# HannesStark/3DInfomax

Hardware: AMD Instinct MI355X
Metric: molecules/sec pretraining step (PNA+Net3D, QM9-50k); PNA-agg HBM GB/s vs peak (higher is better)
Workload: dtype f32

## Files before the change

3dinfomax_amd/csrc/bn.hip:

```cpp
#include <stdlib.h>

#include <atomic>

#include "common.h"
#include "peer.h"

namespace i3d {

constexpr int MAX_PARTIAL_BLOCKS = 256;
static int partial_blocks() { return MAX_PARTIAL_BLOCKS; }
constexpr int RU = 4;

struct Chunking {
    int tpr;
    int rl;
    int rpb;
    int nblk;
    int ncolblk;
    int cv;
    int V;
};

static Chunking make_chunking(int rows, int feat) {
    Chunking c;
    c.V = (feat % 4 == 0) ? 4 : 1;
    c.cv = feat / c.V;
    c.tpr = c.cv < 256 ? c.cv : 256;
    c.rl = 256 / c.tpr;
    c.ncolblk = cdiv(c.cv, c.tpr);
    int rpb = cdiv(rows, partial_blocks());
    int min_rpb = c.rl * 4;
    if (rpb < min_rpb) rpb = min_rpb;
    c.rpb = rpb;
    c.nblk = rows > 0 ? cdiv(rows, rpb) : 0;
    return c;
}

enum { MODE_STATS = 0, MODE_BN_BWD = 1, MODE_COLSUM = 2 };

template <bool GA = true>
__device__ __forceinline__ float stats_pivot(float v, int act) {
    if (act == I3D_ACT_RELU || act == I3D_ACT_LEAKY_RELU) return fmaxf(v, 0.f);
    return GA ? apply_act(v, act) : v;
}

constexpr int FIN_COLS = 8, FIN_LANES = 32;
constexpr int WS_HEADER = 128;

struct Final {
    int kind;
    int feat, rows, act;
    float eps, momentum;
    const float* pre_row0;
    float* mean;
    float* invstd;
    float* running_mean;
    float* running_var;
    float* out1;
    float* out2;
    double* sums_out;
    long long* batches_tracked;
    unsigned* counters;
    int peer_on;
    float* g1;
    float* g2;
    float* ginv;
    PeerDev peer;
};

__device__ __forceinline__ float ld_agent(const float* p) {
    return __hip_atomic_load(p, __ATOMIC_RELAXED, __HIP_MEMORY_SCOPE_AGENT);
}
__device__ __forceinline__ void st_agent(float* p, float v) {
    __hip_atomic_store(p, v, __ATOMIC_RELAXED, __HIP_MEMORY_SCOPE_AGENT);
}

template <bool GA>
__device__ __forceinline__ void finalize_column(const Final& f, int c, double s1, double s2) {
    if (f.kind == 0) {
        const double shift = (double)stats_pivot<GA>(f.pre_row0[c], f.act);
        const double n = (double)f.rows;
        if (f.sums_out != nullptr) {
            f.sums_out[c] = s1 + n * shift;
            f.sums_out[f.feat + c] = s2 + 2.0 * shift * s1 + n * shift * shift;
// ... 856 lines not shown

__global__ void __launch_bounds__(256) act_fwd_kernel(const float* __restrict__ x, long n, int act, float* __restrict__ y) {
    I3D_CHAIN_PRIO();
    for (long t = (long)blockIdx.x * blockDim.x + threadIdx.x; t < n; t += (long)gridDim.x * blockDim.x)
        y[t] = apply_act_any(x[t], act);
}

__global__ void __launch_bounds__(256)
act_bwd_kernel(const float* __restrict__ gy, const float* __restrict__ x, long n, int act, float* __restrict__ gx) {
    I3D_CHAIN_PRIO();
    for (long t = (long)blockIdx.x * blockDim.x + threadIdx.x; t < n; t += (long)gridDim.x * blockDim.x)
        gx[t] = gy[t] * act_grad_any(x[t], act);
}

__global__ void __launch_bounds__(256) add_inplace_kernel(float* __restrict__ dst, const float* __restrict__ src, long n) {
    I3D_CHAIN_PRIO();
    for (long t = (long)blockIdx.x * blockDim.x + threadIdx.x; t < n; t += (long)gridDim.x * blockDim.x) dst[t] += src[t];
}

__global__ void __launch_bounds__(256) add_kernel(const float* __restrict__ a, const float* __restrict__ b, long n,
                                                  float* __restrict__ out) {
    I3D_CHAIN_PRIO();
    for (long t = (long)blockIdx.x * blockDim.x + threadIdx.x; t < n; t += (long)gridDim.x * blockDim.x) out[t] = a[t] + b[t];
}

__global__ void __launch_bounds__(256) mul_kernel(const float* __restrict__ a, const float* __restrict__ b, long n, float* out) {
    I3D_CHAIN_PRIO();
    for (long t = (long)blockIdx.x * blockDim.x + threadIdx.x; t < n; t += (long)gridDim.x * blockDim.x) out[t] = a[t] * b[t];
}

__global__ void __launch_bounds__(256) broadcast_row_kernel(const float* __restrict__ row, long rows, int feat,
                                                            float* __restrict__ out) {
    I3D_CHAIN_PRIO();
    const long n = rows * feat;
    for (long t = (long)blockIdx.x * blockDim.x + threadIdx.x; t < n; t += (long)gridDim.x * blockDim.x) out[t] = row[t % feat];
}

static int grid_for(long items) {
    long b = (items + 255) / 256;
    if (b > 256 * 16) b = 256 * 16;
    if (b < 1) b = 1;
    return (int)b;
}

static bool fused_final() {
    static const bool on = [] { const char* e = getenv("I3D_FUSED_FINAL"); return e == nullptr || e[0] != '0'; }();
    return on;
}

static float* partial_of(void* workspace) { return (float*)((char*)workspace + WS_HEADER); }

static bool peer_fits(int feat) { return 6L * feat <= PEER_PAYLOAD_WORDS; }

static Final stats_final_desc(void* workspace, const float* pre, int act, int rows, int feat, float eps, float momentum,
                              float* mean, float* invstd, float* running_mean, float* running_var, double* sums_out,
                              long long* batches_tracked = nullptr) {
    Final f = {};
    f.batches_tracked = batches_tracked;
    f.kind = 0; f.feat = feat; f.rows = rows; f.act = act; f.eps = eps; f.momentum = momentum; f.pre_row0 = pre;
    f.mean = mean; f.invstd = invstd; f.running_mean = running_mean; f.running_var = running_var; f.sums_out = sums_out;
    f.counters = fused_final() ? (unsigned*)workspace : nullptr;
    return f;
}

static Final pair_final_desc(void* workspace, int feat, float* out1, float* out2, double* sums_out) {
    Final f = {};
    f.kind = 1; f.feat = feat; f.out1 = out1; f.out2 = out2; f.sums_out = sums_out;
    f.counters = fused_final() ? (unsigned*)workspace : nullptr;
    return f;
}

static int g_one_launch = [] { const char* e = getenv("I3D_BN_BWD_ONE_LAUNCH"); return (e == nullptr || e[0] != '0') ? 1 : 0; }();
static std::atomic<unsigned> g_fused_tag{0};

static long two_pass_workspace_bytes(int feat) {
    return WS_HEADER + (long)MAX_PARTIAL_BLOCKS * 2 * feat * sizeof(float) + 4 * (long)feat * sizeof(double) + 64;
}

static bool one_launch_shape(int rows, int feat) {
    return rows > 0 && feat > 0 && feat % 4 == 0 && feat <= 2048 &&
           (long)rows <= (long)FUSED_MAX_BLOCKS * (FUSED_THREADS / (feat / 4)) * FUSED_MAX_RPT;
}

static bool bn_bwd_one_launch(const BwdApplyArgs& b, int rows, int feat, void* workspace, float* grad_beta, float* grad_gamma, hipStream_t s) {
    if (!g_one_launch || !fused_final() || !one_launch_shape(rows, feat) || b.pre != nullptr || b.grad_pre == nullptr) return false;
    if (b.ld_out % 4 != 0 || ((((uintptr_t)b.grad_y) | ((uintptr_t)b.grad_pre)) & 15) != 0 || (((uintptr_t)b.x) & (b.x_bf16 ? 7 : 15)) != 0)
        return false;
    FusedBwdGeom ge;
    ge.tpr = feat / 4;
    ge.rl = FUSED_THREADS / ge.tpr;
    int G = cdiv(rows, ge.rl);
    if (G > FUSED_MAX_BLOCKS) G = FUSED_MAX_BLOCKS;
    ge.rpb = cdiv(rows, G);
    G = cdiv(rows, ge.rpb);
    unsigned tag = ++g_fused_tag;
    if (tag == 0) tag = ++g_fused_tag;
    ge.tag = tag;
    unsigned long long* tpart = (unsigned long long*)((char*)workspace + ((two_pass_workspace_bytes(feat) + 63) & ~63L));
    unsigned long long* tfinal = tpart + (long)FUSED_MAX_BLOCKS * 2 * feat;
    const int rpt = cdiv(ge.rpb, ge.rl);
    const bool ga = !(relu_class(b.act) && relu_class(b.post_act));
#define I3D_LAUNCH_FUSED(R)                                                                                                        \
    do {                                                                                                                             \
        if (ga) hipLaunchKernelGGL((bn_bwd_fused_kernel<R, true>), dim3(G), dim3(FUSED_THREADS), 0, s, b, rows, ge, tpart, tfinal,  \
                                   grad_beta, grad_gamma);                                                                           \
        else hipLaunchKernelGGL((bn_bwd_fused_kernel<R, false>), dim3(G), dim3(FUSED_THREADS), 0, s, b, rows, ge, tpart, tfinal,    \
                                grad_beta, grad_gamma);                                                                              \
    } while (0)
    if (rpt <= 2) I3D_LAUNCH_FUSED(2);
    else if (rpt <= 4) I3D_LAUNCH_FUSED(4);
    else if (rpt <= 6) I3D_LAUNCH_FUSED(6);
    else if (rpt == 7) I3D_LAUNCH_FUSED(7);
    else I3D_LAUNCH_FUSED(8);
#undef I3D_LAUNCH_FUSED
    return true;
}

template <int MODE>
static void launch_reduction(const ReduceArgs& g, const Chunking& ch, const Final& f, hipStream_t s) {
    dim3 grid(ch.nblk, ch.ncolblk);
    const bool ga = !(relu_class(g.act) && relu_class(g.post_act));
    if (ch.V == 4) {
        if (ga) hipLaunchKernelGGL((colreduce_partial_kernel<MODE, 4, true>), grid, dim3(256), 0, s, g, ch, f);
        else hipLaunchKernelGGL((colreduce_partial_kernel<MODE, 4, false>), grid, dim3(256), 0, s, g, ch, f);
    } else {
        if (ga) hipLaunchKernelGGL((colreduce_partial_kernel<MODE, 1, true>), grid, dim3(256), 0, s, g, ch, f);
        else hipLaunchKernelGGL((colreduce_partial_kernel<MODE, 1, false>), grid, dim3(256), 0, s, g, ch, f);
    }
    if (f.counters != nullptr) return;
    if (f.kind == 0)
        hipLaunchKernelGGL(stats_final_kernel, dim3(cdiv(f.feat, FIN_COLS)), dim3(256), 0, s, g.partial, ch.nblk, f.pre_row0,
                           f.act, f.rows, f.feat, f.eps, f.momentum, f.mean, f.invstd, f.running_mean, f.running_var, f.sums_out,
                           f.batches_tracked);
    else
        hipLaunchKernelGGL(pair_final_kernel, dim3(cdiv(f.feat, FIN_COLS)), dim3(256), 0, s, g.partial, ch.nblk, f.feat, f.out1,
                           f.out2, f.sums_out);
}

__global__ void set_double_kernel(double* p, double v) { *p = v; }

}

using namespace i3d;

extern "C" long i3d_colreduce_workspace_bytes(int rows, int feat) {
    (void)rows;
    return ((two_pass_workspace_bytes(feat) + 63) & ~63L) + ((long)FUSED_MAX_BLOCKS + 1) * 2 * feat * 8;
}

extern "C" int i3d_act_stats_fwd(const float* pre, int rows, int feat, int act, float* x, float eps, float momentum,
                                 float* mean, float* invstd, float* running_mean, float* running_var,
                                 double* sums_out, void* workspace, void* stream) {
    return i3d_act_stats_fwd_counted(pre, rows, feat, act, x, eps, momentum, mean, invstd, running_mean, running_var,
                                     sums_out, nullptr, workspace, stream);
}

extern "C" int i3d_act_stats_fwd_counted(const float* pre, int rows, int feat, int act, float* x, float eps, float momentum,
                                         float* mean, float* invstd, float* running_mean, float* running_var,
                                         double* sums_out, long long* num_batches_tracked, void* workspace, void* stream) {
    I3D_CHECK_ARG(rows > 0 && feat > 0, "rows > 0 and feat > 0 required");
    I3D_CHECK_ARG(workspace != nullptr, "workspace required");
    I3D_CHECK_ARG(fused_act(act), "this activation exists as an elementwise pass only (i3d_act_fwd / i3d_act_bwd)");
    hipStream_t s = (hipStream_t)stream;
    if (const I3dCollectives* coll = sums_out == nullptr ? collectives() : nullptr) {
        PeerCtx* pc = peer_active(stream);
        if (pc != nullptr && fused_final() && peer_fits(feat)) {
            Chunking ch = make_chunking(rows, feat);
            ReduceArgs g = {};
            g.a = pre; g.out = x; g.rows = rows; g.feat = feat; g.act = act; g.post_act = I3D_ACT_NONE;
            g.partial = partial_of(workspace);
            Final f = stats_final_desc(workspace, pre, act, rows, feat, eps, momentum, mean, invstd, running_mean, running_var, nullptr,
                                       num_batches_tracked);
            f.peer_on = 1;
            if (int rc = peer_next(pc, &f.peer)) return rc;
            launch_reduction<MODE_STATS>(g, ch, f, s);
            I3D_CHECK_LAUNCH();
            return I3D_OK;
// ... 9 lines not shown
        hipLaunchKernelGGL(stats_from_sums_kernel, dim3(cdiv(feat, 128)), dim3(128), 0, s, s64, feat, eps, momentum, mean, invstd,
                           running_mean, running_var, num_batches_tracked);
        I3D_CHECK_LAUNCH();
        return I3D_OK;
    }
    Chunking ch = make_chunking(rows, feat);
    ReduceArgs g = {};
    g.a = pre; g.out = x; g.rows = rows; g.feat = feat; g.act = act; g.post_act = I3D_ACT_NONE;
    g.partial = partial_of(workspace);
    launch_reduction<MODE_STATS>(g, ch, stats_final_desc(workspace, pre, act, rows, feat, eps, momentum, mean, invstd,
                                                         running_mean, running_var, sums_out, num_batches_tracked), s);
    I3D_CHECK_LAUNCH();
    return I3D_OK;
}

extern "C" int i3d_bn_finalize_stats(const double* sums, int feat, float eps, float momentum, float* mean,
                                     float* invstd, float* running_mean, float* running_var, void* stream) {
    I3D_CHECK_ARG(feat > 0, "feat > 0 required");
    hipLaunchKernelGGL(stats_from_sums_kernel, dim3(cdiv(feat, 128)), dim3(128), 0, (hipStream_t)stream, sums, feat, eps,
                       momentum, mean, invstd, running_mean, running_var);
    I3D_CHECK_LAUNCH();
    return I3D_OK;
}

static int bn_apply_common(const float* x, int rows, int feat, const float* mean, const float* invstd_or_var,
                           const float* gamma, const float* beta, int post_act, const float* residual, float* y,
                           int eval_mode, float eps, void* stream) {
    if (rows == 0) return I3D_OK;
    ApplyArgs g;
    g.x = x; g.mean = mean; g.invstd = invstd_or_var; g.gamma = gamma; g.beta = beta; g.residual = residual; g.y = y;
    g.feat = feat; g.post_act = post_act; g.eval_mode = eval_mode; g.eps = eps;
    hipStream_t s = (hipStream_t)stream;
    g.items = 0;
    const int V = feat % 4 == 0 ? 4 : 1;
    const RowTiling rt = make_row_tiling(feat, V);
    dim3 grid(cdiv(rows, rt.rl * RU), rt.ncolblk);
    const bool ga = !relu_class(post_act);
    if (V == 4) {
        if (ga) hipLaunchKernelGGL((bn_apply_kernel<4, true>), grid, dim3(256), 0, s, g, rt, rows);
        else hipLaunchKernelGGL((bn_apply_kernel<4, false>), grid, dim3(256), 0, s, g, rt, rows);
    } else {
        if (ga) hipLaunchKernelGGL((bn_apply_kernel<1, true>), grid, dim3(256), 0, s, g, rt, rows);
        else hipLaunchKernelGGL((bn_apply_kernel<1, false>), grid, dim3(256), 0, s, g, rt, rows);
    }
    return I3D_OK;
}

extern "C" int i3d_bn_apply_fwd(const float* x, int rows, int feat, const float* mean, const float* invstd,
                                const float* gamma, const float* beta, int post_act, const float* residual, float* y,
                                void* stream) {
    I3D_CHECK_ARG(rows >= 0 && feat > 0, "bad shape");
    I3D_CHECK_ARG(fused_act(post_act), "this activation exists as an elementwise pass only (i3d_act_fwd / i3d_act_bwd)");
    bn_apply_common(x, rows, feat, mean, invstd, gamma, beta, post_act, residual, y, 0, 0.f, stream);
    I3D_CHECK_LAUNCH();
    return I3D_OK;
}

extern "C" int i3d_bn_eval_fwd(const float* x, int rows, int feat, const float* running_mean,
                               const float* running_var, float eps, const float* gamma, const float* beta,
                               int post_act, const float* residual, float* y, void* stream) {
    I3D_CHECK_ARG(rows >= 0 && feat > 0, "bad shape");
    I3D_CHECK_ARG(fused_act(post_act), "this activation exists as an elementwise pass only (i3d_act_fwd / i3d_act_bwd)");
    bn_apply_common(x, rows, feat, running_mean, running_var, gamma, beta, post_act, residual, y, 1, eps, stream);
    I3D_CHECK_LAUNCH();
    return I3D_OK;
}

static void launch_bwd_apply(BwdApplyArgs& g, int rows, int feat, hipStream_t s) {
    g.items = 0;
    const int V = feat % 4 == 0 ? 4 : 1;
    const RowTiling rt = make_row_tiling(feat, V);
    dim3 grid(cdiv(rows, rt.rl * RU), rt.ncolblk);
    const bool ga = !(relu_class(g.act) && relu_class(g.post_act));
    if (V == 4) {
        if (ga) hipLaunchKernelGGL((bn_bwd_apply_kernel<4, true>), grid, dim3(256), 0, s, g, rt, rows);
        else hipLaunchKernelGGL((bn_bwd_apply_kernel<4, false>), grid, dim3(256), 0, s, g, rt, rows);
    } else {
        if (ga) hipLaunchKernelGGL((bn_bwd_apply_kernel<1, true>), grid, dim3(256), 0, s, g, rt, rows);
        else hipLaunchKernelGGL((bn_bwd_apply_kernel<1, false>), grid, dim3(256), 0, s, g, rt, rows);
    }
}

extern "C" int i3d_bn_bwd_one_launch_supported(int rows, int feat) {
    return g_one_launch && fused_final() && collectives() == nullptr && one_launch_shape(rows, feat) ? 1 : 0;
}

extern "C" int i3d_set_bn_bwd_one_launch(int on) {
    const int was = g_one_launch;
    g_one_launch = on ? 1 : 0;
    return was;
}

extern "C" long i3d_bn_bias_partial_floats(int feat) { return (long)MAX_PARTIAL_BLOCKS * 2 * feat; }

static thread_local int g_x_bf16 = 0;
static thread_local const EdgeSums* g_edge_sums = nullptr;
static thread_local int g_sums_ready = 0;

static int bn_bwd_impl(const float* grad_y, const float* x, const float* pre, int rows, int feat, int act,
                       int post_act, const float* mean, const float* invstd, const float* gamma,
                       const float* beta, float* grad_gamma, float* grad_beta, float* grad_pre,
                       float* grad_bias, double* sums_out, const double* sums_in, long total_rows,
                       void* workspace, int ld_out, void* stream) {
    I3D_CHECK_ARG(rows > 0 && feat > 0, "rows > 0 and feat > 0 required");
    I3D_CHECK_ARG(workspace != nullptr, "workspace required");
    I3D_CHECK_ARG(act == I3D_ACT_NONE || act == I3D_ACT_RELU || act == I3D_ACT_LEAKY_RELU || pre != nullptr, "pre required for this activation");
    I3D_CHECK_ARG(fused_act(act) && fused_act(post_act), "this activation exists as an elementwise pass only (i3d_act_fwd / i3d_act_bwd)");
    hipStream_t s = (hipStream_t)stream;
    if (const I3dCollectives* coll = (sums_out == nullptr && sums_in == nullptr) ? collectives() : nullptr) {
        PeerCtx* pc = peer_active(stream);
        if (pc != nullptr && fused_final() && peer_fits(feat)) {
            Chunking ch = make_chunking(rows, feat);
            float* partial = partial_of(workspace);
            float* tmp = partial + (long)MAX_PARTIAL_BLOCKS * 2 * feat;
            ReduceArgs g = {};
            g.a = grad_y; g.b = x; g.mean = mean; g.invstd = invstd; g.gamma = gamma; g.beta = beta;
            g.rows = rows; g.feat = feat; g.act = act; g.post_act = post_act; g.partial = partial;
            g.b_bf16 = g_x_bf16;
            Final f = pair_final_desc(workspace, feat, grad_beta, grad_gamma, nullptr);
            f.rows = rows; f.peer_on = 1; f.g1 = tmp; f.g2 = tmp + feat; f.ginv = tmp + 2 * feat;
            if (int rc = peer_next(pc, &f.peer)) return rc;
            launch_reduction<MODE_BN_BWD>(g, ch, f, s);
            I3D_CHECK_LAUNCH();
            g_sums_ready = 1;
            const int rc = bn_bwd_impl(grad_y, x, pre, rows, feat, act, post_act, mean, invstd, gamma, beta, grad_gamma, grad_beta,
                                       grad_pre, grad_bias, nullptr, (const double*)tmp , 0, workspace,
                                       ld_out, stream);
            g_sums_ready = 0;
            return rc;
        }
        I3D_CHECK_ARG((pc ? peer_scratch_bytes(pc) : coll->scratch_bytes) >= (long)(2 * feat + 1) * 8, "collective scratch too small");
        double* s64 = (double*)(pc ? peer_scratch(pc) : coll->scratch);
        int rc = bn_bwd_impl(grad_y, x, pre, rows, feat, act, post_act, mean, invstd, gamma, beta, grad_gamma, grad_beta,
                             nullptr, nullptr, s64, nullptr, rows, workspace, ld_out, stream);
        if (rc != I3D_OK) return rc;
        if (pc != nullptr) {
            float* tmp = partial_of(workspace) + (long)MAX_PARTIAL_BLOCKS * 2 * feat;
            rc = peer_sum_f64(pc, s64, 2 * feat, 1, (double)rows, nullptr, tmp, tmp + 2 * feat, stream);
            if (rc != I3D_OK) return rc;
            g_sums_ready = 1;
            rc = bn_bwd_impl(grad_y, x, pre, rows, feat, act, post_act, mean, invstd, gamma, beta, grad_gamma, grad_beta,
                             grad_pre, grad_bias, nullptr, s64, 0, workspace, ld_out, stream);
            g_sums_ready = 0;
            return rc;
        }
        hipLaunchKernelGGL(set_double_kernel, dim3(1), dim3(1), 0, s, s64 + 2 * feat, (double)rows);
        I3D_CHECK_LAUNCH();
        rc = coll->all_reduce_f64(coll->user, s64, 2 * feat + 1, stream);
        if (rc != I3D_OK) return rc;
        return bn_bwd_impl(grad_y, x, pre, rows, feat, act, post_act, mean, invstd, gamma, beta, grad_gamma, grad_beta,
                           grad_pre, grad_bias, nullptr, s64, 0, workspace, ld_out, stream);
    }
    Chunking ch = make_chunking(rows, feat);
    float* partial = partial_of(workspace);
    if (sums_in == nullptr && sums_out == nullptr && g_edge_sums == nullptr && grad_pre != nullptr &&
        (grad_bias == nullptr || act == I3D_ACT_NONE)) {
        BwdApplyArgs b = {};
        b.grad_y = grad_y; b.x = x; b.pre = relu_class(act) ? nullptr : pre; b.mean = mean; b.invstd = invstd; b.gamma = gamma;
        b.beta = beta; b.sum_dy = grad_beta; b.sum_dy_xhat = grad_gamma; b.inv_n = 1.f / (float)rows; b.grad_pre = grad_pre;
        b.ld_out = ld_out; b.feat = feat; b.act = act; b.post_act = post_act; b.zero_out = grad_bias; b.x_bf16 = g_x_bf16;
        if (bn_bwd_one_launch(b, rows, feat, workspace, grad_beta, grad_gamma, s)) {
            I3D_CHECK_LAUNCH();
            return I3D_OK;
        }
    }
    if (sums_in == nullptr) {
        ReduceArgs g = {};
        g.a = grad_y; g.b = x; g.mean = mean; g.invstd = invstd; g.gamma = gamma; g.beta = beta;
// ... 209 lines not shown
```

3dinfomax_amd/csrc/common.h:

```cpp
#pragma once
#include <hip/hip_runtime.h>
#include <stdint.h>
#include <stdio.h>

#include "../../include/infomax3d_hip.h"

namespace i3d {

void set_error(const char* fmt, ...);

const I3dCollectives* collectives();

#define I3D_CHECK_ARG(cond, msg)                                  \
    do {                                                          \
        if (!(cond)) {                                            \
            i3d::set_error("%s: invalid argument: %s", __func__, msg); \
            return I3D_ERR_INVALID;                               \
        }                                                         \
    } while (0)

#define I3D_CHECK_LAUNCH()                                                       \
    do {                                                                         \
        hipError_t e_ = hipGetLastError();                                       \
        if (e_ != hipSuccess) {                                                  \
            i3d::set_error("%s: launch failed: %s", __func__, hipGetErrorString(e_)); \
            return I3D_ERR_LAUNCH;                                               \
        }                                                                        \
    } while (0)

static inline int cdiv(long a, long b) { return (int)((a + b - 1) / b); }

constexpr int WAVE = 64;

#ifndef I3D_CHAIN_PRIO_LEVEL
#define I3D_CHAIN_PRIO_LEVEL 3
#endif
#define I3D_CHAIN_PRIO() __builtin_amdgcn_s_setprio(I3D_CHAIN_PRIO_LEVEL)

__device__ __forceinline__ float apply_act(float x, int act) {
    switch (act) {
        case I3D_ACT_RELU: return x > 0.f ? x : 0.f;
        case I3D_ACT_SILU: return x / (1.f + __expf(-x));
        case I3D_ACT_SIGMOID: return 1.f / (1.f + __expf(-x));
        case I3D_ACT_LEAKY_RELU: return x > 0.f ? x : 0.01f * x;
        default: return x;
    }
}

__device__ __forceinline__ float act_grad(float x, int act) {
    switch (act) {
        case I3D_ACT_RELU: return x > 0.f ? 1.f : 0.f;
        case I3D_ACT_SILU: {
            float s = 1.f / (1.f + __expf(-x));
            return s * (1.f + x * (1.f - s));
        }
        case I3D_ACT_SIGMOID: {
            float s = 1.f / (1.f + __expf(-x));
            return s * (1.f - s);
        }
        case I3D_ACT_LEAKY_RELU: return x > 0.f ? 1.f : 0.01f;
        default: return 1.f;
    }
}

inline bool relu_class(int act) { return act == I3D_ACT_NONE || act == I3D_ACT_RELU || act == I3D_ACT_LEAKY_RELU; }
template <bool GA>
__device__ __forceinline__ float apply_act_c(float x, int act) {
    if (GA) return apply_act(x, act);
    return act == I3D_ACT_RELU ? (x > 0.f ? x : 0.f) : (act == I3D_ACT_LEAKY_RELU ? (x > 0.f ? x : 0.01f * x) : x);
}
template <bool GA>
__device__ __forceinline__ float act_grad_c(float x, int act) {
    if (GA) return act_grad(x, act);
    return act == I3D_ACT_RELU ? (x > 0.f ? 1.f : 0.f) : (act == I3D_ACT_LEAKY_RELU ? (x > 0.f ? 1.f : 0.01f) : 1.f);
}

__device__ __forceinline__ float apply_act_any(float x, int act) {
    switch (act) {
        case I3D_ACT_TANH: return tanhf(x);
        case I3D_ACT_ELU: return x > 0.f ? x : expm1f(x);
        case I3D_ACT_SELU: return 1.0507009873554804934193349852946f * (x > 0.f ? x : 1.6732632423543772848170429916717f * expm1f(x));
        case I3D_ACT_SOFTPLUS: return x > 20.f ? x : log1pf(expf(x));
        default: return apply_act(x, act);
    }
}

__device__ __forceinline__ float act_grad_any(float x, int act) {
    switch (act) {
        case I3D_ACT_TANH: {
            const float t = tanhf(x);
            return 1.f - t * t;
        }
        case I3D_ACT_ELU: return x > 0.f ? 1.f : expf(x);
        case I3D_ACT_SELU: return 1.0507009873554804934193349852946f * (x > 0.f ? 1.f : 1.6732632423543772848170429916717f * expf(x));
        case I3D_ACT_SOFTPLUS: return x > 20.f ? 1.f : 1.f / (1.f + expf(-x));
        default: return act_grad(x, act);
    }
}

inline bool fused_act(int act) { return act >= I3D_ACT_NONE && act <= I3D_ACT_LEAKY_RELU; }

__device__ __forceinline__ double block_sum_f64(double v, double* sm) {
    for (int o = 32; o > 0; o >>= 1) v += __shfl_xor(v, o);
    const int lane = threadIdx.x & 63, w = threadIdx.x >> 6;
    __syncthreads();
    if (lane == 0) sm[w] = v;
    __syncthreads();
    return ((sm[0] + sm[1]) + sm[2]) + sm[3];
}

void k4_time_next_launch(void* start, void* stop);

}
// ... 1 lines not shown
```

3dinfomax_amd/csrc/composite.hip:

```cpp
#include "common.h"

using namespace i3d;

#define TRY(call)                 \
    do {                          \
        int rc_ = (call);         \
        if (rc_ != I3D_OK) return rc_; \
    } while (0)

#include <algorithm>
#include <cstdlib>
#include <cstring>
#include <map>
#include <mutex>
#include <utility>

namespace {

struct Aux {
    hipStream_t s = nullptr;
    hipEvent_t fork = nullptr, join = nullptr;
};

Aux* aux_for(hipStream_t main) {
// ... 175 lines not shown

static int edge_fc_bn_bwd_wgrad(const I3dEdgeFcArgs* a, void* wst) {
    TRY(edge_fc_bn_bwd_wgrad_p(a, wst));
    return edge_fc_bn_bwd_wgrad_q(a, wst);
}

extern "C" int i3d_edge_fc_bn_bwd(const I3dEdgeFcArgs* a, void* stream) {
    I3D_CHECK_ARG(a != nullptr && a->num_edges > 0 && a->num_nodes > 0, "bad arguments");
    TRY(edge_fc_bn_bwd_chain(a, stream));
    TRY(edge_fc_bn_bwd_wgrad(a, stream));
    return edge_fc_bn_bwd_dgrad(a, stream);
}

extern "C" int i3d_grouped_fc_bn_fwd(const I3dGroupedFcArgs* a, void* stream) {
    I3D_CHECK_ARG(a != nullptr && a->num_nodes > 0 && a->n_groups > 0, "bad arguments");
    const int Fh = a->f_h, Fo = a->f_out, A = a->agg_width, N = a->num_nodes;
    float* lin = a->pre_keep ? a->pre_keep : a->xact;
    TRY(i3d_gemm_f32(0, 1, N, Fo, Fh, a->h, Fh, a->W, a->ldw, lin, Fo, a->bias, 0, stream));
    TRY(i3d_pna_combine_weights_fwd(a->W, a->ldw, Fh, Fo, A, a->n_groups, a->n_scalers, a->coef, a->WD, stream));
    TRY(i3d_gemm_f32_grouped(1, a->m_padded, Fo, A, a->agg, A, N, a->deg_rows, a->deg_tile_group, a->WD, A, (long)Fo * A, lin,
                             Fo, 1, stream));
    return tail_fwd(&a->tail, N, Fo, lin, a->xact, a->residual, a->y, stream);
}

static int grouped_fc_bn_bwd_chain(const I3dGroupedFcArgs* a, void* stream, int grad_h_accumulate = 0) {
    const int Fh = a->f_h, Fo = a->f_out, A = a->agg_width, N = a->num_nodes;
    TRY(tail_bwd(&a->tail, N, Fo, a->grad_y, a->xact, a->pre_keep, a->grad_gamma, a->grad_beta, a->grad_pre, a->grad_bias,
                 stream));
    TRY(i3d_gemm_f32(0, 0, N, Fh, Fo, a->grad_pre, Fo, a->W, a->ldw, a->grad_h, Fh, nullptr, grad_h_accumulate, stream));
    return i3d_gemm_f32_grouped(0, a->m_padded, A, Fo, a->grad_pre, Fo, N, a->deg_rows, a->deg_tile_group, a->WD, A,
                                (long)Fo * A, a->grad_agg, A, 0, stream);
}

static int grouped_fc_bn_bwd_wgrad(const I3dGroupedFcArgs* a, void* wst) {
    const int Fh = a->f_h, Fo = a->f_out, A = a->agg_width, N = a->num_nodes;
    TRY(i3d_gemm_f32_ws(1, 0, Fo, Fh, N, a->grad_pre, Fo, a->h, Fh, a->grad_W, a->ldw, nullptr, 0, a->tail.gemm_workspace,
                        a->tail.gemm_workspace_bytes, wst));
    TRY(i3d_gemm_f32_rowsubset_multi(Fo, A, a->n_groups, a->group_start, a->group_count, a->grad_pre, Fo, a->agg, A,
                                     a->deg_rows, N, a->grad_WD, (long)Fo * A, A, 0, -1, 0, a->tail.gemm_workspace,
                                     a->tail.gemm_workspace_bytes, wst));
    return i3d_pna_combine_weights_bwd(a->grad_WD, a->ldw, Fh, Fo, A, a->n_groups, a->n_scalers, a->coef, a->grad_W, wst);
}

extern "C" int i3d_grouped_fc_bn_bwd(const I3dGroupedFcArgs* a, void* stream) {
    I3D_CHECK_ARG(a != nullptr && a->num_nodes > 0 && a->n_groups > 0, "bad arguments");
    TRY(grouped_fc_bn_bwd_chain(a, stream));
    return grouped_fc_bn_bwd_wgrad(a, stream);
}

static bool merge_h_ok(const I3dPnaLayerArgs* a) {
    return a->merge_h && a->fused_bn && a->n_post_extra == 0 && a->Wcat != nullptr && a->bcat != nullptr && a->PL != nullptr &&
           a->post.f_h == a->edge.f_h && a->post.pre_keep == nullptr;
}

static int pack_layer_weights(const I3dPnaLayerArgs* a, void* stream) {
    const I3dEdgeFcArgs* e = &a->edge;
    const I3dGroupedFcArgs* p = &a->post;
    TRY(i3d_pna_pack_h_weights(e->W, e->ldw, e->f_out, p->W, p->ldw, p->f_out, p->bias, e->f_h, a->Wcat, a->bcat, stream));
    I3dPanelPack w[8];
    int n = 0;
    const int WL = 2 * e->f_out + p->f_out;
    if (a->Wcat_panel != nullptr) w[n++] = I3dPanelPack{a->Wcat, e->f_h, WL, e->f_h, 1, a->Wcat_panel};
    if (a->Wcat_dgrad_panel != nullptr) w[n++] = I3dPanelPack{a->Wcat, e->f_h, e->f_h, WL, 0, a->Wcat_dgrad_panel};
    for (int i = 0; i < a->n_pre_extra && n + 2 <= 8; ++i) {
        const I3dFcArgs* c = &a->pre[i];
        if (c->W_dgrad_panel != nullptr) w[n++] = I3dPanelPack{c->W, c->ldw, c->f_in, c->f_out, 0, c->W_dgrad_panel};
        if (c->W_fwd_panel != nullptr) w[n++] = I3dPanelPack{c->W, c->ldw, c->f_out, c->f_in, 1, c->W_fwd_panel};
    }
    if (n > 0) TRY(i3d_panel_pack_multi(w, n, stream));
    return I3D_OK;
}

static bool edge_bias_on_chain(const I3dPnaLayerArgs* a) {
    return a->wgrad_split != 0;
}

static bool edge_bwd_fused_ok(const I3dPnaLayerArgs* a) {
    const I3dEdgeFcArgs* e = &a->edge;
    return merge_h_ok(a) && a->DL != nullptr && e->pre_keep == nullptr && relu_class(e->tail.act) && e->tail.post_act == I3D_ACT_NONE &&
           e->f_out % 4 == 0 && e->f_out <= 512 && a->post.f_out % 4 == 0 && e->out_ptr != nullptr && e->out_epos != nullptr &&
           a->edge_bias_partial != nullptr && e->grad_bias != nullptr;
}

static int pna_layer_wgrad_multi(const I3dPnaLayerArgs* a, void* wst, bool dry_run, int part = 0) {
    static const bool on = [] { const char* e = getenv("I3D_WGRAD_MULTI"); return e == nullptr || e[0] != '0'; }();
    const I3dEdgeFcArgs* e = &a->edge;
    const I3dGroupedFcArgs* g = &a->post;
    if (!on || a->n_post_extra != 0 || e->q == nullptr || e->q_rows <= 0) return 0;
    const int Fh = e->f_h, Fo = e->f_out, N = e->num_nodes, E = e->num_edges, A = g->agg_width;
    const bool merged = merge_h_ok(a) && a->DL != nullptr;
    const int WL = 2 * Fo + g->f_out;
    const float* dlin = merged ? a->DL + 2 * Fo : g->grad_pre;
    const int ld_dlin = merged ? WL : g->f_out;
    const float* dP = merged ? a->DL : e->grad_P;
    const int ld_dP = merged ? WL : 2 * Fo;
    constexpr int MAX_PROBLEMS = 40, MAX_OUTPUTS = 8, MAX_GROUPS = 32, MAX_SCALERS = 4;
    I3dWgradProblem pr[MAX_PROBLEMS];
    I3dWgradOutput out[MAX_OUTPUTS];
    float coef[MAX_GROUPS * MAX_SCALERS];
    const int fixed_problems = 3 + (a->n_pre_extra > 0 ? a->n_pre_extra : 0);
    if (g->n_scalers > MAX_SCALERS || g->n_scalers < 0 || fixed_problems >= MAX_PROBLEMS || 4 + a->n_pre_extra > MAX_OUTPUTS) return 0;
    const int max_group_problems = MAX_PROBLEMS - fixed_problems < MAX_GROUPS ? MAX_PROBLEMS - fixed_problems : MAX_GROUPS;
    std::memset(pr, 0, sizeof(pr));
    std::memset(out, 0, sizeof(out));
    int np = 0, no = 0;
    auto problem = [&](const float* Ap, int lda, int M, const float* Bp, int ldb, int Nn, long rows_total, const int* rows,
                       int k_begin, int k_count) {
        I3dWgradProblem& p = pr[np++];
        p.A = Ap; p.B = Bp; p.rows = rows; p.rows_total = rows_total; p.lda = lda; p.ldb = ldb; p.M = M; p.N = Nn;
        p.k_begin = k_begin; p.k_count = k_count;
    };
    const bool do_post = part != 2, do_pre = part != 1;
    if (do_post) {
        out[no].kind = I3D_WGRAD_PLAIN; out[no].n_groups = 1; out[no].first_problem = np; out[no].C = g->grad_W; out[no].ldc = g->ldw;
        ++no;
        problem(dlin, ld_dlin, g->f_out, g->h, Fh, Fh, N, nullptr, 0, N);
    }
    if (do_post) {
        I3dWgradOutput& o = out[no];
        o.kind = I3D_WGRAD_COMBINE; o.first_problem = np; o.C = g->grad_W + Fh; o.ldc = g->ldw;
        o.n_scalers = g->n_scalers; o.scaler_stride = A; o.coef = coef;
        int ng = 0;
        for (int k = 0; k < g->n_groups; ++k) {
            bool any = false;
            for (int s = 0; s < g->n_scalers; ++s) any = any || g->coef[k * g->n_scalers + s] != 0.f;
            if (!any || g->group_count[k] == 0) continue;
            if (ng >= max_group_problems) return 0;
            for (int s = 0; s < g->n_scalers; ++s) coef[ng * g->n_scalers + s] = g->coef[k * g->n_scalers + s];
            problem(dlin, ld_dlin, g->f_out, g->agg, A, A, N, g->deg_rows, g->group_start[k], g->group_count[k]);
            ++ng;
        }
        if (ng == 0) return 0;
        o.n_groups = ng;
        ++no;
    }
    for (int i = a->n_pre_extra - 1; i >= 0 && do_pre; --i) {
        const I3dFcArgs* c = &a->pre[i];
        I3dWgradOutput& o = out[no++];
        o.n_groups = 1; o.first_problem = np; o.C = c->grad_W; o.ldc = c->ldw;
        if (a->fused_bn) { o.kind = I3D_WGRAD_BN; o.aff = a->aff[i]; o.row = c->grad_bias; }
        else o.kind = I3D_WGRAD_PLAIN;
        problem(c->grad_pre, c->f_out, c->f_out, c->x, c->f_in, c->f_in, c->rows, nullptr, 0, c->rows);
    }
    if (do_pre) {
        I3dWgradOutput& o = out[no++];
        o.kind = I3D_WGRAD_PLAIN; o.n_groups = 1; o.first_problem = np; o.C = e->grad_W; o.ldc = e->ldw;
        o.c_split = Fo; o.c_delta = (long)Fh - (long)Fo * e->ldw;
        problem(dP, ld_dP, 2 * Fo, e->h, Fh, Fh, N, nullptr, 0, N);
    }
    if (do_pre) {
        I3dWgradOutput& o = out[no++];
        o.kind = I3D_WGRAD_PLAIN; o.n_groups = 1; o.first_problem = np; o.C = e->grad_Q; o.ldc = Fo;
        problem(e->onehot, e->v_pad, e->v_pad, e->grad_pre, Fo, Fo, E, nullptr, 0, E);
    }
    void* ws = e->tail.gemm_workspace;
    const long wsb = e->tail.gemm_workspace_bytes;
    if (ws == nullptr || !i3d_wgrad_multi_supported(pr, np, out, no) || i3d_wgrad_multi_min_workspace_bytes(pr, np) > wsb) return 0;
    if (dry_run) return 1;
    if (do_pre && edge_bwd_fused_ok(a) && !edge_bias_on_chain(a))
        TRY(i3d_colsum_strided(a->DL + Fo, 2 * Fo + a->post.f_out, N, Fo, e->grad_bias, a->edge_bias_partial, wst));
    TRY(i3d_wgrad_multi(pr, np, out, no, ws, wsb, wst));
    if (!do_pre) return 1;
    const int V = e->q_rows;
    TRY(i3d_gemm_f32_ws(1, 0, Fo, e->f_q, V, e->grad_Q, Fo, e->q, e->f_q, e->grad_W + 2 * Fh, e->ldw, nullptr, 0, ws, wsb, wst));
    if (e->grad_q != nullptr)
        TRY(i3d_gemm_f32(0, 0, V, e->f_q, Fo, e->grad_Q, Fo, e->W + 2 * Fh, e->ldw, e->grad_q, e->f_q, nullptr, e->grad_q_accumulate, wst));
    return 1;
}

static bool wgrad_multi_layer_ok(const I3dPnaLayerArgs* a);

static bool simple_act(int act) { return act == I3D_ACT_NONE || act == I3D_ACT_RELU || act == I3D_ACT_LEAKY_RELU; }

static int finalize_stats(const I3dBnTail* t, const float* partial, int tiles, int feat, float* aff, void* stream,
                          int eval_mode = 0) {
    if (eval_mode) return I3D_OK;
    return i3d_bn_finalize_partials(partial, tiles, feat, t->eps, t->momentum, t->gamma, t->beta, t->mean, t->invstd,
                                    t->running_mean, t->running_var, t->num_batches_tracked, aff, stream);
}

static int pna_layer_fwd_fused(const I3dPnaLayerArgs* a, void* stream) {
    const I3dEdgeFcArgs* e = &a->edge;
    const int Fh = e->f_h, Fo = e->f_out, N = e->num_nodes, E = e->num_edges;
    I3D_CHECK_ARG(a->stats_ws != nullptr && a->n_post_extra == 0 && e->pre_keep == nullptr && simple_act(e->tail.act) &&
                      e->tail.post_act == I3D_ACT_NONE && a->aff[0] != nullptr, "fused BatchNorm: unsupported block shape");
    const I3dGroupedFcArgs* pg = &a->post;
    const bool merged = merge_h_ok(a);
    const int WL = 2 * Fo + pg->f_out;
    const float* P = e->P;
    int ldp = 2 * Fo;
    if (merged) {
        if (!a->weights_ready) TRY(pack_layer_weights(a, stream));
        if (panel_ok(a->Wcat_panel, Fh, WL))
            TRY(i3d_panel_gemm(N, WL, Fh, e->h, Fh, a->Wcat_panel, a->PL, WL, a->bcat, 0, stream));
        else
            TRY(i3d_gemm_f32(0, 1, N, WL, Fh, e->h, Fh, a->Wcat, Fh, a->PL, WL, a->bcat, 0, stream));
        P = a->PL;
        ldp = WL;
    } else {
        const long wdelta = (long)Fh - (long)Fo * e->ldw, wview = (long)(Fo - 1) * e->ldw + 2 * Fh;
        TRY(i3d_gemm_f32_blocks(0, 1, N, 2 * Fo, Fh, e->h, Fh, e->W, e->ldw, Fo, wdelta, wview, e->P, 2 * Fo, 0, 0, 0, nullptr, 0,
                                stream));
    }
    if (e->q != nullptr && !a->weights_ready)
        TRY(i3d_gemm_f32(0, 1, e->q_rows > 0 ? e->q_rows : E, Fo, e->f_q, e->q, e->f_q, e->W + 2 * Fh, e->ldw, e->Q, Fo,
                         nullptr, 0, stream));
    TRY(i3d_edge_combine_act_stats(P, ldp, e->q ? e->Q : nullptr, e->q_rows > 0 ? e->q_code : nullptr, e->bias, e->src_s,
                                   e->dst_s, E, Fo, e->tail.act, e->xact, a->stats_ws, stream));
    TRY(finalize_stats(&e->tail, a->stats_ws, cdiv(E, i3d_edge_stats_rows_per_tile(Fo)), Fo, a->aff[0], stream, a->eval_mode));
    const float* x = e->xact;
    const float* aff = a->aff[0];
    int f_in = Fo;
    for (int i = 0; i < a->n_pre_extra; ++i) {
        const I3dFcArgs* c = &a->pre[i];
        I3D_CHECK_ARG(c->pre_keep == nullptr && simple_act(c->tail.act) && c->tail.post_act == I3D_ACT_NONE &&
                          a->aff[i + 1] != nullptr && c->rows == E && c->f_in == f_in, "fused BatchNorm: unsupported block shape");
        int stat_tiles = cdiv(E, 64);
        if (a->msg_bf16 && i == a->n_pre_extra - 1)
            TRY(i3d_gemm_f32_fused_bf16out(E, c->f_out, f_in, x, f_in, E, c->W, c->ldw, c->xact, c->f_out, c->bias, aff, c->tail.act,
                                           a->stats_ws, stream));
        else if (merged && panel_ok(c->W_fwd_panel, f_in, c->f_out) && (((uintptr_t)x | (uintptr_t)c->xact | (uintptr_t)aff) & 15) == 0) {
            TRY(i3d_panel_gemm_fused(E, c->f_out, f_in, x, f_in, c->W_fwd_panel, c->xact, c->f_out, c->bias, aff, c->tail.act, a->stats_ws,
                                     stream));
            stat_tiles = i3d_panel_stats_tiles(E);
        } else
            TRY(i3d_gemm_f32_fused(E, c->f_out, f_in, x, f_in, E, c->W, c->ldw, c->xact, c->f_out, c->bias, 0, aff, c->tail.act,
                                   a->stats_ws, nullptr, nullptr, 0, stream));
        TRY(finalize_stats(&c->tail, a->stats_ws, stat_tiles, c->f_out, a->aff[i + 1], stream, a->eval_mode));
        x = c->xact;
        aff = a->aff[i + 1];
        f_in = c->f_out;
    }
    if (a->agg_event_start != nullptr && a->agg_event_stop != nullptr) k4_time_next_launch(a->agg_event_start, a->agg_event_stop);
    TRY(i3d_pna_aggregate_fwd_ex(x, a->msg_bf16 && a->n_pre_extra > 0, aff, e->in_ptr, N, f_in, a->aggregators, a->n_aggregators, a->scalers,
                                 a->n_scalers, a->force_scalers, a->avg_d_log, const_cast<float*>(a->post.agg), stream));
    const I3dGroupedFcArgs* p = &a->post;
    I3D_CHECK_ARG(p->pre_keep == nullptr && simple_act(p->tail.act), "fused BatchNorm: unsupported block shape");
    const int A = p->agg_width, Fp = p->f_out;
    if (!merged) TRY(i3d_gemm_f32(0, 1, N, Fp, p->f_h, p->h, p->f_h, p->W, p->ldw, p->xact, Fp, p->bias, 0, stream));
    if (!a->weights_ready)
        TRY(i3d_pna_combine_weights_fwd(p->W, p->ldw, p->f_h, Fp, A, p->n_groups, p->n_scalers, p->coef, p->WD, stream));
    TRY(i3d_gemm_f32_fused_src(p->m_padded, Fp, A, p->agg, A, N, p->WD, A, p->xact, Fp, merged ? a->PL + 2 * Fo : nullptr, WL,
                               nullptr, 1, nullptr, p->tail.act, a->stats_ws, p->deg_rows, p->deg_tile_group, (long)Fp * A, stream));
    if (a->eval_mode)
        return i3d_bn_eval_fwd(p->xact, N, Fp, p->tail.running_mean, p->tail.running_var, p->tail.eps, p->tail.gamma, p->tail.beta,
                               p->tail.post_act, p->residual, p->y, stream);
    TRY(finalize_stats(&p->tail, a->stats_ws, p->m_padded / 64, Fp, nullptr, stream));
    return i3d_bn_apply_fwd(p->xact, N, Fp, p->tail.mean, p->tail.invstd, p->tail.gamma, p->tail.beta, p->tail.post_act,
                            p->residual, p->y, stream);
}

extern "C" int i3d_pna_layer_weights_fwd(const I3dPnaLayerArgs* a, void* stream) {
    I3D_CHECK_ARG(a != nullptr && a->fused_bn, "fused_bn layers only");
    const I3dEdgeFcArgs* e = &a->edge;
    const I3dGroupedFcArgs* p = &a->post;
    if (e->q != nullptr)
        TRY(i3d_gemm_f32(0, 1, e->q_rows > 0 ? e->q_rows : e->num_edges, e->f_out, e->f_q, e->q, e->f_q, e->W + 2 * e->f_h, e->ldw,
                         e->Q, e->f_out, nullptr, 0, stream));
    if (merge_h_ok(a)) TRY(pack_layer_weights(a, stream));
    return i3d_pna_combine_weights_fwd(p->W, p->ldw, p->f_h, p->f_out, p->agg_width, p->n_groups, p->n_scalers, p->coef, p->WD,
                                       stream);
}

extern "C" int i3d_wgrad_stream_fork(void* stream, void** side) {
    I3D_CHECK_ARG(side != nullptr, "null");
    *side = fork_wgrad(aux_for((hipStream_t)stream), stream);
    return I3D_OK;
}

extern "C" int i3d_wgrad_stream_peek(void* stream, void** side) {
    I3D_CHECK_ARG(side != nullptr, "null");
    Aux* x = aux_for((hipStream_t)stream);
    *side = x != nullptr ? (void*)x->s : stream;
    return I3D_OK;
}

extern "C" long i3d_pna_layer_stats_floats(int num_nodes, int num_edges, int m_padded, int f) {
    (void)num_nodes;
    const int rpt = i3d_edge_stats_rows_per_tile(f);
    long tiles = cdiv(num_edges, rpt > 0 ? rpt : 1);
    tiles = std::max<long>(tiles, 2L * cdiv(num_edges, 64));
    tiles = std::max<long>(tiles, m_padded / 64 + 1);
    return tiles * 3 * f;
}

extern "C" int i3d_pna_layer_fwd(const I3dPnaLayerArgs* a, void* stream) {
    I3D_CHECK_ARG(a != nullptr && a->n_pre_extra >= 0 && a->n_pre_extra <= I3D_MAX_EXTRA_FC && a->n_post_extra >= 0 &&
                      a->n_post_extra <= I3D_MAX_EXTRA_FC, "bad arguments");
    if (a->fused_bn) return pna_layer_fwd_fused(a, stream);
    TRY(i3d_edge_fc_bn_fwd(&a->edge, stream));
    for (int i = 0; i < a->n_pre_extra; ++i) TRY(i3d_fc_bn_fwd(&a->pre[i], stream));
    if (a->agg_event_start != nullptr && a->agg_event_stop != nullptr) k4_time_next_launch(a->agg_event_start, a->agg_event_stop);
    TRY(i3d_pna_aggregate_fwd(a->msg, a->edge.in_ptr, a->edge.num_nodes, a->edge.f_out, a->aggregators, a->n_aggregators,
                              a->scalers, a->n_scalers, a->force_scalers, a->avg_d_log, const_cast<float*>(a->post.agg), stream));
    TRY(i3d_grouped_fc_bn_fwd(&a->post, stream));
    for (int i = 0; i < a->n_post_extra; ++i) TRY(i3d_fc_bn_fwd(&a->postx[i], stream));
    return I3D_OK;
}

extern "C" int i3d_pna_layer_bwd(const I3dPnaLayerArgs* a, void* stream) {
    I3D_CHECK_ARG(a != nullptr && a->n_pre_extra >= 0 && a->n_pre_extra <= I3D_MAX_EXTRA_FC && a->n_post_extra >= 0 &&
                      a->n_post_extra <= I3D_MAX_EXTRA_FC, "bad arguments");
    Aux* x = aux_for((hipStream_t)stream);
    for (int i = a->n_post_extra - 1; i >= 0; --i) TRY(fc_bn_bwd_chain(&a->postx[i], stream));
    const bool inplace = a->residual && a->post.grad_h == a->grad_out && a->n_post_extra == 0;
    I3D_CHECK_ARG(a->post.grad_h != a->grad_out || inplace, "grad_h may alias grad_out only for a residual layer without extra blocks");
    const bool multi = wgrad_multi_layer_ok(a);
    const bool merged = multi && merge_h_ok(a) && a->DL != nullptr;
    const long n = (long)a->edge.num_nodes * a->edge.f_h;
    if (merged) {
        const I3dGroupedFcArgs* g = &a->post;
        const int WLb = 2 * a->edge.f_out + g->f_out;
        float* dlin = a->DL + 2 * a->edge.f_out;
        TRY(i3d_bn_bwd_strided(g->grad_y, g->xact, g->pre_keep, g->num_nodes, g->f_out, g->tail.act, g->tail.post_act, g->tail.mean,
                               g->tail.invstd, g->tail.gamma, g->tail.beta, g->grad_gamma, g->grad_beta, dlin, WLb, g->grad_bias,
                               g->tail.workspace, stream));
        TRY(i3d_gemm_f32_grouped(0, g->m_padded, g->agg_width, g->f_out, dlin, WLb, g->num_nodes, g->deg_rows, g->deg_tile_group, g->WD,
                                 g->agg_width, (long)g->f_out * g->agg_width, g->grad_agg, g->agg_width, 0, stream));
    } else {
        TRY(grouped_fc_bn_bwd_chain(&a->post, stream, inplace ? 1 : 0));
        if (a->residual && !inplace) TRY(i3d_add_inplace(a->post.grad_h, a->grad_out, n, stream));
    }
    void* wst = stream;
    if (multi && a->wgrad_split) {
        wst = fork_wgrad(x, stream);
        const int took = pna_layer_wgrad_multi(a, wst, false, 1);
        if (took < 0) return took;
        I3D_CHECK_ARG(took == 1, "weight-gradient launch refused a layer it had accepted");
    }
    if (!multi) {
        wst = fork_wgrad(x, stream);
        TRY(grouped_fc_bn_bwd_wgrad(&a->post, wst));
        for (int i = a->n_post_extra - 1; i >= 0; --i) TRY(fc_bn_bwd_wgrad(&a->postx[i], wst));
    }
    const float* msg_aff = a->fused_bn ? a->aff[a->n_pre_extra] : nullptr;
    const int f_msg = a->n_pre_extra > 0 ? a->pre[a->n_pre_extra - 1].f_out : a->edge.f_out;
    const int msg16 = a->fused_bn && a->msg_bf16 && a->n_pre_extra > 0;
    TRY(i3d_pna_aggregate_bwd_ex(a->post.grad_agg, a->msg, msg16, msg_aff, a->edge.in_ptr, a->edge.num_nodes, f_msg, a->aggregators,
                                 a->n_aggregators, a->scalers, a->n_scalers, a->force_scalers, a->avg_d_log, a->grad_msg, stream));
    for (int i = a->n_pre_extra - 1; i >= 0; --i) TRY(fc_bn_bwd_chain(&a->pre[i], stream, msg16 && i == a->n_pre_extra - 1));
    const bool edge_fused = multi && merged && edge_bwd_fused_ok(a);
    if (edge_fused) {
        const I3dEdgeFcArgs* e = &a->edge;
        const int WLb = 2 * e->f_out + a->post.f_out;
        if (i3d_bn_bwd_one_launch_supported(e->num_edges, e->f_out)) {
            TRY(i3d_bn_bwd_strided(e->grad_y, e->xact, nullptr, e->num_edges, e->f_out, e->tail.act, I3D_ACT_NONE, e->tail.mean, e->tail.invstd,
                                   e->tail.gamma, e->tail.beta, e->grad_gamma, e->grad_beta, e->grad_pre, e->f_out, nullptr,
                                   e->tail.workspace, stream));
            TRY(i3d_segment_sum_pair(e->grad_pre, e->f_out, e->out_ptr, e->out_epos, a->DL, e->in_ptr, nullptr, a->DL + e->f_out,
                                     e->num_nodes, e->f_out, WLb, stream));
        } else
        TRY(i3d_bn_bwd_edge_sums(e->grad_y, e->xact, e->num_edges, e->f_out, e->tail.act, e->tail.mean, e->tail.invstd, e->tail.gamma,
                                 e->tail.beta, e->grad_gamma, e->grad_beta, e->grad_pre, e->in_ptr, e->out_ptr, e->out_epos, e->num_nodes,
                                 a->DL, a->DL + e->f_out, WLb, e->tail.workspace, stream));
    } else {
        TRY(edge_fc_bn_bwd_tail(&a->edge, stream));
    }
    if (multi) {
        if (edge_fused) {
        } else if (merged) {
            const I3dEdgeFcArgs* e = &a->edge;
            const int WLb = 2 * e->f_out + a->post.f_out;
            TRY(i3d_segment_sum_pair(e->grad_pre, e->f_out, e->out_ptr, e->out_epos, a->DL, e->in_ptr, nullptr, a->DL + e->f_out,
                                     e->num_nodes, e->f_out, WLb, stream));
        } else {
            TRY(edge_fc_bn_bwd_sums(&a->edge, stream));
        }
        wst = fork_wgrad(x, stream);
        const int took = pna_layer_wgrad_multi(a, wst, false, a->wgrad_split ? 2 : 0);
        if (took < 0) return took;
        I3D_CHECK_ARG(took == 1, "weight-gradient launch refused a layer it had accepted");
    } else {
        TRY(edge_fc_bn_bwd_sums(&a->edge, stream));
        wst = fork_wgrad(x, stream);
        for (int i = a->n_pre_extra - 1; i >= 0; --i) TRY(fc_bn_bwd_wgrad(&a->pre[i], wst, a->fused_bn ? a->aff[i] : nullptr));
        TRY(edge_fc_bn_bwd_wgrad(&a->edge, wst));
    }
    if (merged) {
        const int WLb = 2 * a->edge.f_out + a->post.f_out;
        if (panel_ok(a->Wcat_dgrad_panel, WLb, a->edge.f_h, 1024) && (((uintptr_t)a->DL | (uintptr_t)a->post.grad_h) & 15) == 0)
            TRY(i3d_panel_gemm(a->edge.num_nodes, a->edge.f_h, WLb, a->DL, WLb, a->Wcat_dgrad_panel, a->post.grad_h, a->edge.f_h, nullptr,
                               inplace ? 1 : 0, stream));
        else
            TRY(i3d_gemm_f32(0, 0, a->edge.num_nodes, a->edge.f_h, WLb, a->DL, WLb, a->Wcat, a->edge.f_h, a->post.grad_h, a->edge.f_h,
                             nullptr, inplace ? 1 : 0, stream));
        if (a->residual && !inplace) TRY(i3d_add_inplace(a->post.grad_h, a->grad_out, n, stream));
    } else {
        TRY(edge_fc_bn_bwd_dgrad(&a->edge, stream, a->post.grad_h));
    }
    if (edge_fused && edge_bias_on_chain(a)) {
        const int Fo = a->edge.f_out;
        TRY(i3d_colsum_strided(a->DL + Fo, 2 * Fo + a->post.f_out, a->edge.num_nodes, Fo, a->edge.grad_bias, a->edge_bias_partial, stream));
    }
    if (a->defer_join) return I3D_OK;
    return join_wgrad(x, stream);
}

static bool wgrad_multi_layer_ok(const I3dPnaLayerArgs* a) { return pna_layer_wgrad_multi(a, nullptr, true) == 1; }

extern "C" int i3d_wgrad_stream_join(void* stream) { return join_wgrad(aux_for((hipStream_t)stream), stream); }

extern "C" int i3d_event_create(void** event) {
    I3D_CHECK_ARG(event != nullptr, "null");
    hipEvent_t e;
    if (hipEventCreateWithFlags(&e, hipEventDisableSystemFence) != hipSuccess &&
        hipEventCreateWithFlags(&e, hipEventReleaseToDevice) != hipSuccess && hipEventCreate(&e) != hipSuccess) {
        i3d::set_error("hipEventCreate failed");
        return I3D_ERR_LAUNCH;
    }
    *event = (void*)e;
    return I3D_OK;
}

extern "C" int i3d_event_destroy(void* event) {
    if (event != nullptr) (void)hipEventDestroy((hipEvent_t)event);
    return I3D_OK;
}

extern "C" int i3d_event_record(void* event, void* stream) {
    I3D_CHECK_ARG(event != nullptr, "null");
    if (hipEventRecord((hipEvent_t)event, (hipStream_t)stream) != hipSuccess) {
        i3d::set_error("hipEventRecord failed");
        return I3D_ERR_LAUNCH;
    }
    return I3D_OK;
}

extern "C" int i3d_event_elapsed_ms(void* start, void* stop, float* ms) {
    I3D_CHECK_ARG(start != nullptr && stop != nullptr && ms != nullptr, "null");
    if (hipEventElapsedTime(ms, (hipEvent_t)start, (hipEvent_t)stop) != hipSuccess) {
        i3d::set_error("hipEventElapsedTime failed (events not completed?)");
        return I3D_ERR_LAUNCH;
    }
    return I3D_OK;
}
```

3dinfomax_amd/csrc/embedding.hip:

```cpp
#include <stdarg.h>

#include "common.h"

namespace i3d {

static thread_local char g_err[512] = "";

void set_error(const char* fmt, ...) {
    va_list ap;
    va_start(ap, fmt);
    vsnprintf(g_err, sizeof(g_err), fmt, ap);
    va_end(ap);
}

constexpr int MAX_TABLES = 16;
struct Tables {
    const float* t[MAX_TABLES];
};
struct GradTables {
    float* t[MAX_TABLES];
    int dim[MAX_TABLES];
};

template <int V>
// ... 18 lines not shown
        for (int k = 0; k < 4; ++k) {
            const float* p = tabs.t[min(k0 + k, n_cols - 1)] + rows_[k] * feat + c;
            if (V == 4) {
                float4 v = *reinterpret_cast<const float4*>(p);
                a[k][0] = v.x; a[k][1 % V] = v.y; a[k][2 % V] = v.z; a[k][3 % V] = v.w;
            } else {
                a[k][0] = p[0];
            }
        }
#pragma unroll
        for (int k = 0; k < 4; ++k) {
            if (k0 + k < n_cols) {
#pragma unroll
                for (int i = 0; i < V; ++i) acc[i] += a[k][i];
            }
        }
    }
    float* o = out + (long)r * feat + c;
    if (V == 4) *reinterpret_cast<float4*>(o) = make_float4(acc[0], acc[1 % V], acc[2 % V], acc[3 % V]);
    else o[0] = acc[0];
}

__global__ void __launch_bounds__(256)
embedding_sum_bwd_kernel(const int64_t* __restrict__ idx, const int* __restrict__ row_perm, int rows, int n_cols,
                         const float* __restrict__ gout, int feat, GradTables tabs) {
    I3D_CHAIN_PRIO();
    long t = (long)blockIdx.x * blockDim.x + threadIdx.x;
    if (t >= (long)rows * feat) return;
    int r = (int)(t / feat), c = (int)(t - (long)r * feat);
    float g = gout[t];
    const long ir = row_perm ? row_perm[r] : r;
    for (int k = 0; k < n_cols; ++k) {
        long row = idx[ir * n_cols + k];
        unsafeAtomicAdd(tabs.t[k] + row * feat + c, g);
    }
}

constexpr int LDS_TAB_ROWS = 192, LDS_FW = 64;

__global__ void __launch_bounds__(256)
embedding_sum_bwd_lds_kernel(const int64_t* __restrict__ idx, const int* __restrict__ row_perm, int rows, int n_cols,
                             const float* __restrict__ gout, int feat, GradTables tabs, int rows_per_block) {
    I3D_CHAIN_PRIO();
    __shared__ float acc[LDS_TAB_ROWS * LDS_FW];
    __shared__ int off[MAX_TABLES + 1];
    const int t = threadIdx.x;
    if (t == 0) {
        int o = 0;
        for (int k = 0; k < n_cols; ++k) { off[k] = o; o += tabs.dim[k]; }
        off[n_cols] = o;
    }
    for (int i = t; i < LDS_TAB_ROWS * LDS_FW; i += 256) acc[i] = 0.f;
    __syncthreads();
    const int f = t & (LDS_FW - 1), rl = t / LDS_FW;
    const int fg = blockIdx.y * LDS_FW + f;
    const int r0 = blockIdx.x * rows_per_block, r1 = min(rows, r0 + rows_per_block);
    if (fg < feat) {
        for (int r = r0 + rl; r < r1; r += 256 / LDS_FW) {
            const float g = gout[(long)r * feat + fg];
            const long ir = row_perm ? row_perm[r] : r;
            for (int k = 0; k < n_cols; ++k) {
                const int row = off[k] + (int)idx[ir * n_cols + k];
                atomicAdd(&acc[row * LDS_FW + f], g);
            }
        }
    }
    __syncthreads();
    const int total = off[n_cols];
    for (int i = t; i < total * LDS_FW; i += 256) {
        const int row = i / LDS_FW, ff = blockIdx.y * LDS_FW + (i & (LDS_FW - 1));
        const float v = acc[i];
        if (v != 0.f && ff < feat) {
            int k = 0;
            while (row >= off[k + 1]) ++k;
            unsafeAtomicAdd(tabs.t[k] + (long)(row - off[k]) * feat + ff, v);
        }
    }
}

}

using namespace i3d;

extern "C" int i3d_abi_version(void) { return 2; }

extern "C" const char* i3d_last_error(void) { return g_err; }

extern "C" int i3d_embedding_sum_fwd(const int64_t* idx, const int* row_perm, int rows, int n_cols,
                                     const float* const* tables, int feat, float* out, void* stream) {
    I3D_CHECK_ARG(rows >= 0 && feat > 0, "bad shape");
    I3D_CHECK_ARG(n_cols >= 1 && n_cols <= MAX_TABLES, "1..16 tables supported");
    if (rows == 0) return I3D_OK;
    Tables tabs;
    for (int k = 0; k < MAX_TABLES; ++k) tabs.t[k] = k < n_cols ? tables[k] : nullptr;
    bool vec = feat % 4 == 0;
    for (int k = 0; k < n_cols; ++k) vec = vec && (((uintptr_t)tables[k] & 15) == 0);
    hipStream_t s = (hipStream_t)stream;
    if (vec) {
        long items = (long)rows * feat / 4;
        hipLaunchKernelGGL(embedding_sum_fwd_kernel<4>, dim3(cdiv(items, 256)), dim3(256), 0, s, idx, row_perm, rows, n_cols,
                           tabs, feat, out);
    } else {
        long items = (long)rows * feat;
        hipLaunchKernelGGL(embedding_sum_fwd_kernel<1>, dim3(cdiv(items, 256)), dim3(256), 0, s, idx, row_perm, rows, n_cols,
                           tabs, feat, out);
    }
    I3D_CHECK_LAUNCH();
    return I3D_OK;
}

extern "C" int i3d_embedding_sum_bwd(const int64_t* idx, const int* row_perm, int rows, int n_cols,
                                     const float* grad_out, int feat, float* const* grad_tables, const int* dims,
                                     void* stream) {
    I3D_CHECK_ARG(rows >= 0 && feat > 0, "bad shape");
    I3D_CHECK_ARG(n_cols >= 1 && n_cols <= MAX_TABLES, "1..16 tables supported");
    if (rows == 0) return I3D_OK;
    GradTables tabs;
    for (int k = 0; k < MAX_TABLES; ++k) {
        tabs.t[k] = k < n_cols ? grad_tables[k] : nullptr;
        tabs.dim[k] = (k < n_cols && dims) ? dims[k] : 0;
    }
    int total_rows = 0;
    for (int k = 0; k < n_cols; ++k) total_rows += tabs.dim[k];
    if (dims != nullptr && total_rows > 0 && total_rows <= LDS_TAB_ROWS) {
        int rpb = cdiv(rows, 128);
        if (rpb < 32) rpb = 32;
        dim3 grid(cdiv(rows, rpb), cdiv(feat, LDS_FW));
        hipLaunchKernelGGL(embedding_sum_bwd_lds_kernel, grid, dim3(256), 0, (hipStream_t)stream, idx, row_perm, rows,
                           n_cols, grad_out, feat, tabs, rpb);
    } else {
        long items = (long)rows * feat;
        hipLaunchKernelGGL(embedding_sum_bwd_kernel, dim3(cdiv(items, 256)), dim3(256), 0, (hipStream_t)stream, idx,
                           row_perm, rows, n_cols, grad_out, feat, tabs);
    }
    I3D_CHECK_LAUNCH();
    return I3D_OK;
}
```

3dinfomax_amd/csrc/model.hip:

```cpp
#include "common.h"


#include <algorithm>
#include <cmath>
#include <cstdlib>
#include <cstring>
#include <new>
#include <vector>

using namespace i3d;

#define TRY(call)                 \
    do {                          \
        int rc_ = (call);         \
        if (rc_ != I3D_OK) return rc_; \
    } while (0)

namespace {

inline long al4(long n) { return (n + 3) & ~3L; }

struct Bump {
    float* base;
    long used = 0;
// ... 418 lines not shown
                        return I3D_ERR_LAUNCH;
                    }
                }
                TRY(i3d_colsum(gpre_of[i], nullptr, B, p.f_out, p.grad_bias, cws, wst));
            }
        }
        return I3D_OK;
    };
    bool leaves_pending = false;
    if (part != 2) {
        Bump ar(head_buf);
        const float* gy = grad_out;
        for (int i = m.n_head - 1; i >= 0; --i) {
            I3dFcArgs& fc = c->head_args[i];
            const I3dFcParams& p = m.head[i];
            float* gx = ar.take((long)B * p.f_in);
            if (p.gamma != nullptr) {
                set_ws(fc.tail, bn_workspace, gemm_workspace, side_ws_bytes);
                fc.grad_y = gy; fc.grad_pre = ar.take((long)B * p.f_out); fc.grad_x = gx;
                fc.grad_W = p.grad_W; fc.grad_bias = p.grad_bias; fc.grad_gamma = p.grad_gamma; fc.grad_beta = p.grad_beta;
                TRY(i3d_fc_bn_bwd_chain(&fc, stream));
            } else {
                const float* gpre = gy;
                if (p.act != I3D_ACT_NONE) {
                    float* t = ar.take((long)B * p.f_out);
                    TRY(i3d_act_bwd(gy, fc.xact, (long)B * p.f_out, p.act, t, stream));
                    gpre = t;
                }
                TRY(i3d_gemm_f32(0, 0, B, p.f_in, p.f_out, gpre, p.f_out, p.W, p.f_in, gx, p.f_in, nullptr, 0, stream));
                gpre_of[i] = gpre;
            }
            gy = gx;
        }
        constexpr bool leaves_aside = true;
        leaves_pending = leaves_aside && l_hi == L && l_hi > l_lo;
        if (!leaves_pending) TRY(head_leaves(stream));
        TRY(i3d_segment_readout_bwd(gy, c->h[L], b.graph_ptr, B, F, m.readout_ops, m.n_readout, gh[L & 1], stream));
        c->gh_cur = L & 1;
    }
    for (int l = l_hi - 1; l >= l_lo; --l) {
        I3dPnaLayerArgs& a = c->layers[l];
        Bump ar(rest);
        Bump sd(side[l]);
        a.defer_join = 1;
        a.wgrad_split = l == 0 ? 1 : 0;
        const int cur = c->gh_cur, nxt = a.residual ? cur : cur ^ 1;
        const float* grad_in = gh[cur];
        a.grad_out = grad_in;
        I3dGroupedFcArgs& g = a.post;
        const I3dFcParams& pp = m.post[l];
        set_ws(g.tail, bn_workspace, gemm_workspace, side_ws_bytes);
        g.grad_W = pp.grad_W; g.grad_bias = pp.grad_bias; g.grad_gamma = pp.grad_gamma; g.grad_beta = pp.grad_beta;
        g.grad_y = grad_in;
        g.grad_pre = sd.take((long)N * F);
        g.grad_WD = sd.take((long)b.n_groups * F * g.agg_width);
        g.grad_h = gh[nxt];
        g.grad_agg = ar.take((long)N * g.agg_width);
        const int f_msg = a.n_pre_extra > 0 ? a.pre[a.n_pre_extra - 1].f_out : a.edge.f_out;
        a.grad_msg = ar.take((long)E * f_msg);
        const float* gy = a.grad_msg;
        for (int i = a.n_pre_extra - 1; i >= 0; --i) {
            I3dFcArgs& fc = a.pre[i];
            const I3dFcParams& p = m.pre[l][i + 1];
            set_ws(fc.tail, bn_workspace, gemm_workspace, side_ws_bytes);
            fc.grad_W = p.grad_W; fc.grad_bias = p.grad_bias; fc.grad_gamma = p.grad_gamma; fc.grad_beta = p.grad_beta;
            fc.grad_y = gy;
            fc.grad_pre = sd.take((long)E * fc.f_out);
            fc.grad_x = ar.take((long)E * fc.f_in);
            gy = fc.grad_x;
        }
        I3dEdgeFcArgs& e = a.edge;
        const I3dFcParams& p0 = m.pre[l][0];
        set_ws(e.tail, bn_workspace, gemm_workspace, side_ws_bytes);
        e.grad_W = p0.grad_W; e.grad_bias = p0.grad_bias; e.grad_gamma = p0.grad_gamma; e.grad_beta = p0.grad_beta;
        e.grad_y = gy;
        e.grad_pre = sd.take((long)E * e.f_out);
        e.grad_P = sd.take((long)N * 2 * e.f_out);
        a.DL = sd.take((long)N * (2 * e.f_out + F));
        e.grad_h = ar.take((long)N * F);
        e.grad_Q = sd.take((long)b.v_pad * e.f_out);
        a.edge_bias_partial = sd.take(i3d_bn_bias_partial_floats(e.f_out));
        e.grad_q = grad_table;
        e.grad_q_accumulate = (l == L - 1) ? 0 : 1;
        TRY(i3d_pna_layer_bwd(&a, stream));
        c->gh_cur = nxt;
        if (leaves_pending) {
            void* wst = stream;
            TRY(i3d_wgrad_stream_peek(stream, &wst));
            TRY(head_leaves(wst));
            leaves_pending = false;
        }
    }
    if (part == 1) {
        TRY(i3d_wgrad_stream_join(stream));
        return I3D_OK;
    }
    {
        Bump ar(rest);
        int oa = 0, ob = 0;
        for (int k = 0; k < m.n_atom_tables; ++k) oa += m.atom_dims[k];
        for (int k = 0; k < m.n_bond_tables; ++k) ob += m.bond_dims[k];
        const int va = (oa + 31) / 32 * 32, vb = (ob + 31) / 32 * 32;
        float* hot = c->hot_atoms;
        float* hotb = c->hot_bonds;
        if (!c->hot_ready) {
            hot = ar.take((long)N * va);
            hotb = ar.take((long)b.n_comb * vb);
            TRY(encoder_multihot(*c, hot, hotb, stream));
        }
        const bool own_ws = tail_bytes > 0;
        const int oa4 = (oa + 3) / 4 * 4;
        float* atoms_out = oa4 == oa ? m.grad_atom_tables : ar.take((long)oa4 * F);
        auto atom_tables = [&](void* ws, long wsb) -> int {
            TRY(wgrad(oa4, F, N, hot, va, gh[c->gh_cur], F, atoms_out, F, ws, wsb, stream));
            if (atoms_out != m.grad_atom_tables &&
                hipMemcpyAsync(m.grad_atom_tables, atoms_out, (size_t)oa * F * sizeof(float), hipMemcpyDeviceToDevice, (hipStream_t)stream) != hipSuccess) {
                i3d::set_error("i3d_pna_model_bwd: copy of the atom-table gradient failed");
                return I3D_ERR_LAUNCH;
            }
            return I3D_OK;
        };
        if (own_ws) TRY(atom_tables(tail_ws, tail_bytes - 256));
        void* bst = stream;
        constexpr bool bond_aside = true;
        if (bond_aside && own_ws && c->hot_ready) TRY(i3d_wgrad_stream_peek(stream, &bst));
        if (bst != stream)
            TRY(wgrad(ob, F, b.n_comb, hotb, vb, grad_table, F, m.grad_bond_tables, F, gemm_workspace, side_ws_bytes, bst));
        TRY(i3d_wgrad_stream_join(stream));
        if (!own_ws) TRY(atom_tables(gemm_workspace, gemm_workspace_bytes));
        if (bst == stream)
            TRY(wgrad(ob, F, b.n_comb, hotb, vb, grad_table, F, m.grad_bond_tables, F, gemm_workspace, gemm_workspace_bytes, stream));
    }
    return I3D_OK;
}

extern "C" int i3d_pna_model_debug_messages(void* ctx, int layer, float* out, void* stream) {
    I3D_CHECK_ARG(ctx != nullptr && out != nullptr, "null");
    PnaCtx* c = static_cast<PnaCtx*>(ctx);
    I3D_CHECK_ARG(layer >= 0 && layer < c->m.n_layers, "layer out of range");
    const I3dPnaLayerArgs& a = c->layers[layer];
    const int f_msg = a.n_pre_extra > 0 ? a.pre[a.n_pre_extra - 1].f_out : a.edge.f_out;
    return i3d_pna_messages_normalized_ex(a.msg, a.fused_bn && a.msg_bf16 && a.n_pre_extra > 0, a.aff[a.n_pre_extra], a.edge.num_edges, f_msg, out, stream);
}

extern "C" int i3d_pna_model_ctx_free(void* ctx) {
    delete static_cast<PnaCtx*>(ctx);
    return I3D_OK;
}
```

3dinfomax_amd/csrc/wgrad.hip:

```cpp
#include "common.h"

#include <algorithm>
#include <cstdlib>
#include <cstring>

namespace i3d {
namespace {

typedef float floatx4 __attribute__((ext_vector_type(4)));
typedef int intx4 __attribute__((ext_vector_type(4)));
typedef short shortx4 __attribute__((ext_vector_type(4)));
typedef __bf16 bf16x4_t __attribute__((ext_vector_type(4)));

constexpr int PREC_F32 = 0, PREC_BF16 = 1, PREC_BF16X3 = 2;

__device__ __forceinline__ void split4(const float v[4], shortx4& hi, shortx4& lo, const bool want_lo) {
    const bf16x4_t h = {(__bf16)v[0], (__bf16)v[1], (__bf16)v[2], (__bf16)v[3]};
    hi = __builtin_bit_cast(shortx4, h);
    if (want_lo) {
        const bf16x4_t l = {(__bf16)(v[0] - (float)h[0]), (__bf16)(v[1] - (float)h[1]), (__bf16)(v[2] - (float)h[2]),
                            (__bf16)(v[3] - (float)h[3])};
        lo = __builtin_bit_cast(shortx4, l);
    }
}
typedef __attribute__((address_space(3))) void* lds_ptr_t;

constexpr int WG_T = 13;
constexpr int WG_LD = 208;
constexpr int WG_LDP = 256;
constexpr int WG_BK = 16;
constexpr int wg_nst(int prec) { return prec == 0 ? 2 : 3; }
constexpr int WG_UNIT_FLOATS = WG_T * WG_T * 256;
constexpr int WG_MAX_PROBLEMS = 40;
constexpr int WG_MAX_SLICE = 1024;
constexpr int WG_MAX_OUTPUTS = 8;

struct WgProb {
    const float* A;
    const float* B;
    const int* rows;
    unsigned a_bytes, b_bytes;
    int lda, ldb;
    int M, N;
    int mcw, ncw;
    int m_chunks, n_chunks;
    int k_begin, k_end, k_per_slice;
    int unit_begin;
};

struct WgArgs {
    float* slab;
    unsigned long long* stamps;
    int n_problems, n_units;
    WgProb p[WG_MAX_PROBLEMS];
};

__device__ __forceinline__ int xcd_unit(int total) {
    const int id = blockIdx.x;
    const int q = total / 8, r = total % 8, xcd = id % 8;
    return xcd * q + min(xcd, r) + id / 8;
}

#ifdef WG_TIMING
#define WG_STAMP(i) do { if (threadIdx.x == 0) stamps[i] = __builtin_readcyclecounter(); } while (0)
#else
#define WG_STAMP(i) do { } while (0)
#endif

template <int MT, bool NFULL, int PREC>
__device__ __forceinline__ void wgrad_unit(const WgProb& p, const int slice, const int mc, const int nc, float* __restrict__ out,
                                           float* __restrict__ smem, int* __restrict__ kidx, unsigned long long* stamps) {
    WG_STAMP(0);
    constexpr int NQ = MT == WG_T ? 4 : (MT + 3) / 4;
    const int lane = threadIdx.x & 63, wave = __builtin_amdgcn_readfirstlane(threadIdx.x >> 6);
    const int l15 = lane & 15, lk = lane >> 4;
    const int k0 = p.k_begin + slice * p.k_per_slice;
    const int klen = min(p.k_end - k0, p.k_per_slice);
    const int mvalid = min(p.mcw, p.M - mc * p.mcw), nvalid = min(p.ncw, p.N - nc * p.ncw);
    const int mtl = (mvalid + 15) / 16, ntl = NFULL ? WG_T : (nvalid + 15) / 16;

    for (int i = threadIdx.x; i < klen; i += 256) kidx[i] = p.rows != nullptr ? p.rows[k0 + i] : k0 + i;

    const unsigned a_rec = p.a_bytes - (unsigned)(mc * p.mcw) * 4u, b_rec = p.b_bytes - (unsigned)(nc * p.ncw) * 4u;
    const unsigned long long pa = (unsigned long long)(p.A + mc * p.mcw), pb = (unsigned long long)(p.B + nc * p.ncw);
    const intx4 da = {(int)(unsigned)pa, (int)(unsigned)(pa >> 32), (int)a_rec, 0x00020000};
    const intx4 db = {(int)(unsigned)pb, (int)(unsigned)(pb >> 32), (int)b_rec, 0x00020000};
    const int pw = wave & 1;
    const int s4 = lane ^ (pw << 2);
    const bool a_ok = s4 * 4 < mvalid, b_ok = s4 * 4 < nvalid;
    const unsigned lda4 = (unsigned)p.lda * 4u, ldb4 = (unsigned)p.ldb * 4u, col = (unsigned)s4 * 16u;

    float* const As = smem;
    constexpr int NST = wg_nst(PREC);
    float* const Bs = smem + NST * WG_BK * WG_LDP;
    const unsigned as_base = (unsigned)(unsigned long long)(lds_ptr_t)As, bs_base = (unsigned)(unsigned long long)(lds_ptr_t)Bs;
    __syncthreads();

    int rnext[4];
    auto read_rows = [&](int t) {
#pragma unroll
        for (int i = 0; i < 4; ++i) rnext[i] = kidx[min(t * WG_BK + wave + 4 * i, klen - 1)];
    };
    auto issue_piece = [&](int t, int buf, int i) {
        const int kr = wave + 4 * i;
        const int kl = t * WG_BK + kr;
        const bool live = kl < klen && rnext[i] >= 0;
        const unsigned oa = (live && a_ok) ? (unsigned)rnext[i] * lda4 + col : a_rec;
        const unsigned ob = (live && b_ok) ? (unsigned)rnext[i] * ldb4 + col : b_rec;
        const unsigned la = as_base + (unsigned)((buf * WG_BK + kr) * WG_LDP) * 4u;
        const unsigned lb = bs_base + (unsigned)((buf * WG_BK + kr) * WG_LDP) * 4u;
        unsigned keep;
        asm volatile("s_mov_b32 %0, m0\n\ts_mov_b32 m0, %1\n\ts_nop 0\n\tbuffer_load_dwordx4 %2, %3, 0 offen lds\n\t"
                     "s_mov_b32 m0, %4\n\ts_nop 0\n\tbuffer_load_dwordx4 %5, %6, 0 offen lds\n\ts_mov_b32 m0, %0"
                     : "=&s"(keep)
                     : "s"(__builtin_amdgcn_readfirstlane(la)), "v"(oa), "s"(da), "s"(__builtin_amdgcn_readfirstlane(lb)), "v"(ob), "s"(db)
                     : "memory");
    };

    floatx4 acc[3][MT], accx[NQ];
#pragma unroll
    for (int j = 0; j < 3; ++j)
#pragma unroll
        for (int i = 0; i < MT; ++i) acc[j][i] = floatx4{0.f, 0.f, 0.f, 0.f};
#pragma unroll
    for (int q = 0; q < NQ; ++q) accx[q] = floatx4{0.f, 0.f, 0.f, 0.f};

    const int nkt = (klen + WG_BK - 1) / WG_BK;
#pragma unroll
    for (int t0 = 0; t0 < NST - 1; ++t0) {
        read_rows(t0);
#pragma unroll
        for (int i = 0; i < 4; ++i) issue_piece(t0, t0, i);
    }
    if constexpr (NST == 2) asm volatile("s_waitcnt vmcnt(0)" ::: "memory");
    else asm volatile("s_waitcnt vmcnt(8)" ::: "memory");
    __syncthreads();
    WG_STAMP(1);
    const bool extra = ntl == WG_T;
    const int b = lk & 1;
    const int even_off = lk * WG_LDP + l15 + 16 * b, odd_off = lk * WG_LDP + l15 - 16 * b;
    const int own_off = pw ? odd_off : even_off;
    for (int t = 0; t < nkt; ++t) {
        const int cur = t % NST, nxt = (t + NST - 1) % NST;
        read_rows(t + NST - 1);
        const float* as = As + cur * WG_BK * WG_LDP;
        const float* bs = Bs + cur * WG_BK * WG_LDP;
        if constexpr (PREC != PREC_F32) {
            constexpr bool X3 = PREC == PREC_BF16X3;
            auto frag = [&](const float* base, int off, shortx4& hi, shortx4& lo) {
                float v[4];
#pragma unroll
                for (int kk = 0; kk < 4; ++kk) v[kk] = base[kk * 4 * WG_LDP + off];
                split4(v, hi, lo, X3);
            };
            auto fma3 = [&](floatx4& c, const shortx4& bh, const shortx4& bl, const shortx4& ah, const shortx4& al) {
                if constexpr (X3) {
                    c = __builtin_amdgcn_mfma_f32_16x16x16bf16_1k(bl, ah, c, 0, 0, 0);
                    c = __builtin_amdgcn_mfma_f32_16x16x16bf16_1k(bh, al, c, 0, 0, 0);
                }
                c = __builtin_amdgcn_mfma_f32_16x16x16bf16_1k(bh, ah, c, 0, 0, 0);
            };
// ... 22 lines not shown
                        __builtin_amdgcn_sched_barrier(0);
                    }
                }
            }
            if (NFULL || extra) {
#pragma unroll
                for (int q = 0; q < NQ; ++q) {
                    shortx4 xh, xl;
                    if (MT == WG_T && q == 3) frag(as, even_off + 12 * 16, xh, xl);
                    else frag(as, own_off + (wave + 4 * q) * 16, xh, xl);
                    fma3(accx[q], bxh, bxl, xh, xl);
                }
            }
        } else
#pragma unroll
        for (int kk = 0; kk < WG_BK / 4; ++kk) {
            const float* ae = as + kk * 4 * WG_LDP + even_off;
            const float* ao = as + kk * 4 * WG_LDP + odd_off;
            const float* aw = as + kk * 4 * WG_LDP + own_off;
            const float* bw = bs + kk * 4 * WG_LDP + own_off;
            const float* be = bs + kk * 4 * WG_LDP + even_off;
            float af[MT], bf[3], ax[NQ], bx;
#pragma unroll
            for (int i = 0; i < MT; ++i) af[i] = (i & 1) ? ao[i * 16] : ae[i * 16];
#pragma unroll
            for (int j = 0; j < 3; ++j) bf[j] = bw[(wave + 4 * j) * 16];
#pragma unroll
            for (int q = 0; q < NQ; ++q) ax[q] = (MT == WG_T && q == 3) ? ae[12 * 16] : aw[(wave + 4 * q) * 16];
            bx = be[12 * 16];
#pragma unroll
            for (int j = 0; j < 3; ++j) {
                if (NFULL || wave + 4 * j < min(ntl, 12)) {
#pragma unroll
                    for (int i = 0; i < MT; ++i) acc[j][i] = __builtin_amdgcn_mfma_f32_16x16x4f32(bf[j], af[i], acc[j][i], 0, 0, 0);
                }
                if (j == 0) {
                    __builtin_amdgcn_sched_barrier(0);
                    issue_piece(t + NST - 1, nxt, kk);
                    __builtin_amdgcn_sched_barrier(0);
                }
            }
            if (NFULL || extra) {
#pragma unroll
                for (int q = 0; q < NQ; ++q) accx[q] = __builtin_amdgcn_mfma_f32_16x16x4f32(bx, ax[q], accx[q], 0, 0, 0);
            }
        }
        if constexpr (NST == 2) asm volatile("s_waitcnt vmcnt(0)" ::: "memory");
        else asm volatile("s_waitcnt vmcnt(8)" ::: "memory");
        __syncthreads();
    }
    if constexpr (NST > 2) asm volatile("s_waitcnt vmcnt(0)" ::: "memory");

    WG_STAMP(2);
    float4* const o4 = reinterpret_cast<float4*>(out) + lane;
#pragma unroll
    for (int j = 0; j < 3; ++j) {
        const int nt = wave + 4 * j;
        if (nt < min(ntl, 12)) {
#pragma unroll
            for (int i = 0; i < MT; ++i)
                if (i < mtl) o4[(i * WG_T + nt) * 64] = make_float4(acc[j][i][0], acc[j][i][1], acc[j][i][2], acc[j][i][3]);
        }
    }
    if (extra) {
#pragma unroll
        for (int q = 0; q < NQ; ++q) {
            const bool row12 = MT == WG_T && q == 3;
            const int mt = row12 ? 12 : wave + 4 * q;
            if ((!row12 || wave == 0) && mt < min(mtl, row12 ? 13 : 12))
                o4[(mt * WG_T + 12) * 64] = make_float4(accx[q][0], accx[q][1], accx[q][2], accx[q][3]);
        }
    }
}

template <int PREC>
__global__ void __launch_bounds__(256, PREC == 0 ? 2 : 1) wgrad_multi_kernel(const WgArgs a) {
    __shared__ __attribute__((aligned(1024))) float smem[2 * wg_nst(PREC) * WG_BK * WG_LDP];
    __shared__ int kidx[WG_MAX_SLICE];
    const int u = xcd_unit(a.n_units);
    int pi = 0;
    while (pi + 1 < a.n_problems && a.p[pi + 1].unit_begin <= u) ++pi;
    const WgProb& p = a.p[pi];
    const int local = u - p.unit_begin;
    const int nc = local % p.n_chunks, mc = (local / p.n_chunks) % p.m_chunks, slice = local / (p.n_chunks * p.m_chunks);
    float* out = a.slab + (long)u * WG_UNIT_FLOATS;
    const int mvalid = min(p.mcw, p.M - mc * p.mcw), nvalid = min(p.ncw, p.N - nc * p.ncw);
    const int mtl = (mvalid + 15) / 16;
    const bool nfull = nvalid > 192;
#ifdef WG_TIMING
    unsigned long long* stamps = a.stamps + (long)blockIdx.x * 8;
    if (threadIdx.x == 0) { stamps[5] = u; stamps[7] = pi; }
#else
    unsigned long long* stamps = nullptr;
#endif
#define WG_DISPATCH(MTV)                                                          \
    do {                                                                          \
        if (nfull) wgrad_unit<MTV, true, PREC>(p, slice, mc, nc, out, smem, kidx, stamps);  \
        else wgrad_unit<MTV, false, PREC>(p, slice, mc, nc, out, smem, kidx, stamps);       \
    } while (0)
    if (mtl > 7) WG_DISPATCH(13);
    else if (mtl > 4) WG_DISPATCH(7);
    else if (mtl > 2) WG_DISPATCH(4);
    else WG_DISPATCH(2);
#undef WG_DISPATCH
#ifdef WG_TIMING
    __builtin_amdgcn_s_waitcnt(0);
    if (threadIdx.x == 0) stamps[3] = __builtin_readcyclecounter();
#endif
}

struct WgOut {
    int kind, n_groups, first_problem;
    int M, N, mcw, ncw, m_chunks, n_chunks;
    int ldc, c_split, n_scalers;
    long c_delta, scaler_stride;
    float* C;
    const float* aff;
    const float* row;
    long item_begin;
};

struct WgReduceArgs {
    const float* slab;
    int n_outputs;
    long total_items;
    WgOut o[WG_MAX_OUTPUTS];
    int unit_begin[WG_MAX_PROBLEMS];
    int n_slices[WG_MAX_PROBLEMS];
    float coef[32][4];
};

template <int S>
__device__ __forceinline__ void wgrad_reduce_item(const WgReduceArgs& a, const WgOut& o, const long item) {
    const int lane = (int)(item & 63);
    long r = item >> 6;
    const int tile = (int)(r % (WG_T * WG_T));
    r /= WG_T * WG_T;
    const int nc = (int)(r % o.n_chunks), mc = (int)(r / o.n_chunks);
    const int mt = tile / WG_T, nt = tile % WG_T;
    const int ml = mt * 16 + (lane & 15), nl = nt * 16 + 4 * (lane >> 4);
    const int mvalid = min(o.mcw, o.M - mc * o.mcw), nvalid = min(o.ncw, o.N - nc * o.ncw);
    if (ml >= mvalid || nl >= nvalid) return;
    const int m = mc * o.mcw + ml, n = nc * o.ncw + nl;
    float4 tot[S];
#pragma unroll
    for (int s = 0; s < S; ++s) tot[s] = make_float4(0.f, 0.f, 0.f, 0.f);
    for (int g = 0; g < o.n_groups; ++g) {
        const int pi = o.first_problem + g;
        const int zn = a.n_slices[pi];
        const long stride = (long)o.m_chunks * o.n_chunks * WG_UNIT_FLOATS;
        const float* p = a.slab + ((long)a.unit_begin[pi] + (long)mc * o.n_chunks + nc) * WG_UNIT_FLOATS + tile * 256 + lane * 4;
        float4 v = make_float4(0.f, 0.f, 0.f, 0.f);
        constexpr int FL = 8;
        for (int z0 = 0; z0 < zn; z0 += FL) {
            float4 x[FL];
#pragma unroll
            for (int k = 0; k < FL; ++k) x[k] = *reinterpret_cast<const float4*>(p + (long)min(z0 + k, zn - 1) * stride);
#pragma unroll
            for (int k = 0; k < FL; ++k)
                if (z0 + k < zn) { v.x += x[k].x; v.y += x[k].y; v.z += x[k].z; v.w += x[k].w; }
        }
        if (o.kind == I3D_WGRAD_COMBINE) {
#pragma unroll
            for (int s = 0; s < S; ++s) {
                const float c = a.coef[g][s];
                tot[s].x += c * v.x; tot[s].y += c * v.y; tot[s].z += c * v.z; tot[s].w += c * v.w;
            }
        } else {
            tot[0] = v;
        }
    }
    float* c = o.C + (long)m * o.ldc + n + (m >= o.c_split ? o.c_delta : 0);
    if (o.kind == I3D_WGRAD_BN) {
        const float rw = o.row[m];
        const float4 mu = *reinterpret_cast<const float4*>(o.aff + n);
        const float4 sc = *reinterpret_cast<const float4*>(o.aff + o.N + n);
        const float4 sh = *reinterpret_cast<const float4*>(o.aff + 2 * o.N + n);
        tot[0].x = (tot[0].x - rw * mu.x) * sc.x + rw * sh.x;
        tot[0].y = (tot[0].y - rw * mu.y) * sc.y + rw * sh.y;
        tot[0].z = (tot[0].z - rw * mu.z) * sc.z + rw * sh.z;
        tot[0].w = (tot[0].w - rw * mu.w) * sc.w + rw * sh.w;
    }
    if (o.kind == I3D_WGRAD_COMBINE) {
#pragma unroll
        for (int s = 0; s < S; ++s) *reinterpret_cast<float4*>(c + (long)s * o.scaler_stride) = tot[s];
    } else {
        *reinterpret_cast<float4*>(c) = tot[0];
    }
}

__global__ void __launch_bounds__(256) wgrad_reduce_kernel(const WgReduceArgs a) {
    const long item = (long)blockIdx.x * 256 + threadIdx.x;
    if (item >= a.total_items) return;
    int oi = 0;
    while (oi + 1 < a.n_outputs && a.o[oi + 1].item_begin <= item) ++oi;
    const WgOut& o = a.o[oi];
    const long local = item - o.item_begin;
    if (o.kind == I3D_WGRAD_COMBINE) {
        switch (o.n_scalers) {
            case 1: wgrad_reduce_item<1>(a, o, local); break;
            case 2: wgrad_reduce_item<2>(a, o, local); break;
            case 3: wgrad_reduce_item<3>(a, o, local); break;
            default: wgrad_reduce_item<4>(a, o, local); break;
        }
    } else {
        wgrad_reduce_item<1>(a, o, local);
    }
}

int env_int(const char* name, int dflt) {
    const char* e = getenv(name);
    return (e != nullptr && e[0] != 0) ? atoi(e) : dflt;
}

int chunk_width(int n, int& chunks) {
    chunks = cdiv(n, WG_LD);
    return cdiv(cdiv(n, chunks), 4) * 4;
}

}
}

using namespace i3d;

extern "C" int i3d_wgrad_multi_supported(const I3dWgradProblem* problems, int n_problems, const I3dWgradOutput* outputs,
                                         int n_outputs) {
    if (problems == nullptr || outputs == nullptr || n_problems < 1 || n_problems > WG_MAX_PROBLEMS || n_outputs < 1 ||
        n_outputs > WG_MAX_OUTPUTS)
        return 0;
    int combines = 0;
    for (int i = 0; i < n_outputs; ++i) {
        const I3dWgradOutput& o = outputs[i];
        if (o.kind == I3D_WGRAD_COMBINE) {
            ++combines;
            if (o.n_groups < 1 || o.n_groups > 32 || o.n_scalers < 1 || o.n_scalers > 4 || o.coef == nullptr || o.scaler_stride % 4 != 0)
                return 0;
        } else if (o.n_groups != 1) {
            return 0;
        }
        if (o.C == nullptr || o.ldc % 4 != 0 || o.c_delta % 4 != 0 || (((uintptr_t)o.C) & 15) != 0) return 0;
        if (o.kind == I3D_WGRAD_BN && (o.aff == nullptr || o.row == nullptr || (((uintptr_t)o.aff) & 15) != 0)) return 0;
        if (o.first_problem < 0 || o.first_problem + o.n_groups > n_problems) return 0;
    }
    if (combines > 1) return 0;
    for (int i = 0; i < n_problems; ++i) {
        const I3dWgradProblem& p = problems[i];
        if (p.A == nullptr || p.B == nullptr || p.M < 4 || p.N < 4 || p.M % 4 != 0 || p.N % 4 != 0 || p.lda % 4 != 0 ||
            p.ldb % 4 != 0 || p.lda < p.M || p.ldb < p.N || ((((uintptr_t)p.A) | ((uintptr_t)p.B)) & 15) != 0 || p.k_count < 0 ||
            p.rows_total < 1)
            return 0;
        if (((p.rows_total - 1) * p.lda + p.M) * 4 >= (1L << 32) - 16 || ((p.rows_total - 1) * p.ldb + p.N) * 4 >= (1L << 32) - 16)
            return 0;
    }
    return 1;
}

static int problem_kps(const I3dWgradProblem& p, int kps) {
    int mch, nch;
    const int mt = std::min(WG_T, cdiv(chunk_width(p.M, mch), 16)), nt = std::min(WG_T, cdiv(chunk_width(p.N, nch), 16));
    const int mt_code = mt > 7 ? 13 : (mt > 4 ? 7 : (mt > 2 ? 4 : 2));
    const int tiles = mt_code * std::min(nt, 12) + (nt == WG_T ? mt_code : 0);
    const long scaled = (long)kps * WG_T * WG_T / std::max(tiles, WG_T * WG_T * 9 / 20);
    return (int)std::min<long>(WG_MAX_SLICE, scaled / WG_BK * WG_BK);
}

static long plan_units(const I3dWgradProblem* problems, int n, int kps) {
    long u = 0;
    for (int i = 0; i < n; ++i) {
        int mch, nch;
        chunk_width(problems[i].M, mch);
        chunk_width(problems[i].N, nch);
        u += (long)mch * nch * cdiv(problems[i].k_count, problem_kps(problems[i], kps));
    }
    return u;
}

extern "C" long i3d_wgrad_multi_workspace_bytes(int max_units) { return (long)max_units * WG_UNIT_FLOATS * 4; }

extern "C" long i3d_wgrad_multi_min_workspace_bytes(const I3dWgradProblem* problems, int n_problems) {
    if (problems == nullptr || n_problems < 1) return -1;
    return (plan_units(problems, n_problems, WG_MAX_SLICE) + 1) * (long)WG_UNIT_FLOATS * 4 + (1 << 16);
}

extern "C" int i3d_wgrad_multi(const I3dWgradProblem* problems, int n_problems, const I3dWgradOutput* outputs, int n_outputs,
                               void* workspace, long workspace_bytes, void* stream) {
    I3D_CHECK_ARG(i3d_wgrad_multi_supported(problems, n_problems, outputs, n_outputs), "unsupported problem set");
    I3D_CHECK_ARG(workspace != nullptr && (((uintptr_t)workspace) & 15) == 0, "scratch required");
#ifdef WG_TIMING
    const long max_units = (workspace_bytes - (1 << 16)) / ((long)WG_UNIT_FLOATS * 4);
#else
    const long max_units = workspace_bytes / ((long)WG_UNIT_FLOATS * 4);
#endif
    static const int fixed_rows = env_int("I3D_WGRAD_ROWS", 0) / WG_BK * WG_BK;
    static const int target_units = env_int("I3D_WGRAD_UNITS", 256);
    int kps;
    if (fixed_rows > 0) {
        kps = std::min(WG_MAX_SLICE, fixed_rows);
        while (kps < WG_MAX_SLICE && plan_units(problems, n_problems, kps) > max_units) kps = std::min(WG_MAX_SLICE, kps * 2);
    } else {
        const long target = std::min<long>(max_units, target_units);
        int lo = 128 / WG_BK, hi = WG_MAX_SLICE / WG_BK;
        while (lo < hi) {
            const int mid = (lo + hi) / 2;
            if (plan_units(problems, n_problems, mid * WG_BK) <= target) hi = mid;
            else lo = mid + 1;
        }
        kps = lo * WG_BK;
    }
    I3D_CHECK_ARG(plan_units(problems, n_problems, kps) <= max_units, "scratch too small");
    WgArgs a;
    WgReduceArgs r;
    a.slab = (float*)workspace;
    a.stamps = nullptr;
#ifdef WG_TIMING
    a.stamps = (unsigned long long*)((char*)workspace + workspace_bytes - (1 << 16));
#endif
    a.n_problems = n_problems;
    int units = 0;
    for (int i = 0; i < n_problems; ++i) {
        const I3dWgradProblem& s = problems[i];
        WgProb& p = a.p[i];
        p.A = s.A; p.B = s.B; p.rows = s.rows;
        p.a_bytes = (unsigned)(((s.rows_total - 1) * s.lda + s.M) * 4);
        p.b_bytes = (unsigned)(((s.rows_total - 1) * s.ldb + s.N) * 4);
        p.lda = s.lda; p.ldb = s.ldb; p.M = s.M; p.N = s.N;
        p.mcw = chunk_width(s.M, p.m_chunks);
        p.ncw = chunk_width(s.N, p.n_chunks);
        p.k_begin = s.k_begin; p.k_end = s.k_begin + s.k_count;
        const int n_slices = cdiv(s.k_count, problem_kps(s, kps));
        p.k_per_slice = n_slices > 0 ? cdiv(cdiv(s.k_count, n_slices), WG_BK) * WG_BK : WG_BK;
        p.unit_begin = units;
        r.unit_begin[i] = units;
        r.n_slices[i] = s.k_count > 0 ? cdiv(s.k_count, p.k_per_slice) : 0;
        units += p.m_chunks * p.n_chunks * r.n_slices[i];
    }
    I3D_CHECK_ARG(units <= max_units, "scratch too small");
    a.n_units = units;
    hipStream_t st = (hipStream_t)stream;
    if (units > 0) {
        const char* const sb = getenv("I3D_WGRAD_SPLIT_BF16");
        const bool split_bf16 = sb != nullptr && sb[0] == '1';
        const int prec = i3d_get_matmul_precision() != 0 ? PREC_BF16 : (split_bf16 ? PREC_BF16X3 : PREC_F32);
        if (prec == PREC_BF16) hipLaunchKernelGGL(wgrad_multi_kernel<PREC_BF16>, dim3(units), dim3(256), 0, st, a);
        else if (prec == PREC_BF16X3) hipLaunchKernelGGL(wgrad_multi_kernel<PREC_BF16X3>, dim3(units), dim3(256), 0, st, a);
        else hipLaunchKernelGGL(wgrad_multi_kernel<PREC_F32>, dim3(units), dim3(256), 0, st, a);
        I3D_CHECK_LAUNCH();
    }
    r.slab = a.slab;
    r.n_outputs = n_outputs;
    long items = 0;
    std::memset(r.coef, 0, sizeof(r.coef));
    for (int i = 0; i < n_outputs; ++i) {
        const I3dWgradOutput& s = outputs[i];
        const WgProb& p = a.p[s.first_problem];
        WgOut& o = r.o[i];
        o.kind = s.kind; o.n_groups = s.n_groups; o.first_problem = s.first_problem;
        o.M = p.M; o.N = p.N; o.mcw = p.mcw; o.ncw = p.ncw; o.m_chunks = p.m_chunks; o.n_chunks = p.n_chunks;
        for (int g = 1; g < s.n_groups; ++g)
            I3D_CHECK_ARG(a.p[s.first_problem + g].M == p.M && a.p[s.first_problem + g].N == p.N, "groups of one output differ in shape");
        o.ldc = s.ldc; o.c_split = s.c_split > 0 ? s.c_split : 0x7fffffff; o.c_delta = s.c_delta;
        o.n_scalers = s.n_scalers; o.scaler_stride = s.scaler_stride;
        o.C = s.C; o.aff = s.aff; o.row = s.row;
        o.item_begin = items;
        items += (long)p.m_chunks * p.n_chunks * WG_T * WG_T * 64;
        if (s.kind == I3D_WGRAD_COMBINE)
            for (int g = 0; g < s.n_groups; ++g)
                for (int k = 0; k < s.n_scalers; ++k) r.coef[g][k] = s.coef[g * s.n_scalers + k];
    }
    r.total_items = items;
    hipLaunchKernelGGL(wgrad_reduce_kernel, dim3(cdiv(items, 256)), dim3(256), 0, st, r);
    I3D_CHECK_LAUNCH();
    return I3D_OK;
}
```

3dinfomax_amd/ops.py:

```python
import ctypes
import os
import threading

import torch

from . import _lib
from ._lib import ACT, AGG, SCALER, check, int_array, ptr_array

_tls = threading.local()
KERNEL_TIMERS = None


_raw_stream = torch._C._cuda_getCurrentRawStream


def _stream():
    return _raw_stream(torch.cuda.current_device())


def _p(t):
    return t.data_ptr() if t is not None else None


def _chk(t, dtype=torch.float32):
# ... 599 lines not shown
    return out


def panel_gemm_fused(A, packed, N, bias=None, a_aff=None, act=None, want_stats=True):
    _chk(A)
    M, K = A.shape
    L = _lib.load()
    out = torch.empty(M, N, dtype=torch.float32, device=A.device)
    tiles = L.i3d_panel_stats_tiles(M)
    partial = torch.empty(tiles, 3, N, dtype=torch.float32, device=A.device) if want_stats else None
    check(L.i3d_panel_gemm_fused(M, N, K, _p(A), A.stride(0), _p(packed), _p(out), N, _p(bias), _p(a_aff), ACT[act], _p(partial), _stream()),
          'i3d_panel_gemm_fused')
    return out, partial, tiles


def gemm_wgrad_bn(dY, x, grad_bias, aff):
    _chk(dY), _chk(x)
    dW = torch.empty(dY.shape[1], x.shape[1], dtype=torch.float32, device=x.device)
    check(_lib.load().i3d_gemm_f32_wgrad_bn(dY.shape[1], x.shape[1], x.shape[0], _p(dY), dY.shape[1], _p(x), x.shape[1], _p(dW),
                                            x.shape[1], _p(grad_bias), _p(aff), _p(_gemm_workspace(x.device)),
                                            GEMM_WORKSPACE_BYTES, _stream()), 'i3d_gemm_f32_wgrad_bn')
    return dW


def pna_aggregate_fwd_aff(e, aff, in_ptr, num_nodes, aggregators, scalers, avg_d_log, force_scalers=False):
    if e.dtype == torch.bfloat16:
        n_s = len(scalers) if (len(scalers) > 1 or force_scalers) else 1
        out = torch.empty(num_nodes, n_s * len(aggregators) * e.shape[1], dtype=torch.float32, device=e.device)
        check(_lib.load().i3d_pna_aggregate_fwd_ex(e.data_ptr(), 1, _p(aff), _p(in_ptr), num_nodes, e.shape[1], int_array(aggregators),
                                                   len(aggregators), int_array(scalers), len(scalers), int(force_scalers),
                                                   float(avg_d_log), _p(out), _stream()), 'i3d_pna_aggregate_fwd_ex')
        return out
    _chk(e)
    n_s = len(scalers) if (len(scalers) > 1 or force_scalers) else 1
    out = torch.empty(num_nodes, n_s * len(aggregators) * e.shape[1], dtype=torch.float32, device=e.device)
    check(_lib.load().i3d_pna_aggregate_fwd_aff(_p(e), _p(aff), _p(in_ptr), num_nodes, e.shape[1], int_array(aggregators),
                                                len(aggregators), int_array(scalers), len(scalers), int(force_scalers),
                                                float(avg_d_log), _p(out), _stream()), 'i3d_pna_aggregate_fwd_aff')
    return out


def pna_aggregate_bwd_aff(grad_out, e, aff, in_ptr, num_nodes, aggregators, scalers, avg_d_log, force_scalers=False):
    if e.dtype == torch.bfloat16:
        _chk(grad_out)
        ge = torch.empty(e.shape, dtype=torch.float32, device=e.device)
        check(_lib.load().i3d_pna_aggregate_bwd_ex(_p(grad_out), e.data_ptr(), 1, _p(aff), _p(in_ptr), num_nodes, e.shape[1],
                                                   int_array(aggregators), len(aggregators), int_array(scalers), len(scalers),
                                                   int(force_scalers), float(avg_d_log), _p(ge), _stream()), 'i3d_pna_aggregate_bwd_ex')
        return ge
    _chk(grad_out), _chk(e)
    ge = torch.empty_like(e)
    check(_lib.load().i3d_pna_aggregate_bwd_aff(_p(grad_out), _p(e), _p(aff), _p(in_ptr), num_nodes, e.shape[1],
                                                int_array(aggregators), len(aggregators), int_array(scalers), len(scalers),
                                                int(force_scalers), float(avg_d_log), _p(ge), _stream()),
          'i3d_pna_aggregate_bwd_aff')
    return ge


def pna_messages_normalized(e, aff):
    bf16 = e.dtype == torch.bfloat16
    _chk(e, torch.bfloat16 if bf16 else torch.float32)
    out = torch.empty(e.shape, dtype=torch.float32, device=e.device)
    check(_lib.load().i3d_pna_messages_normalized_ex(e.data_ptr(), int(bf16), _p(aff), e.shape[0], e.shape[1], _p(out), _stream()),
          'i3d_pna_messages_normalized_ex')
    return out


WGRAD_PLAIN, WGRAD_BN, WGRAD_COMBINE = (_lib.DEFINES[f'I3D_WGRAD_{k}'] for k in ('PLAIN', 'BN', 'COMBINE'))


def wgrad_multi(problems, outputs):
    L = _lib.load()
    pa = (_lib.WgradProblem * len(problems))()
    keep = []
    for d, p in zip(problems, pa):
        A, B = _chk(d['A']), _chk(d['B'])
        p.A, p.B = A.data_ptr(), B.data_ptr()
        p.rows = d['rows'].data_ptr() if d.get('rows') is not None else None
        p.rows_total = A.shape[0]
        p.lda, p.ldb = d.get('lda', A.shape[1]), d.get('ldb', B.shape[1])
        p.M, p.N = d.get('M', A.shape[1]), d.get('N', B.shape[1])
        p.k_begin = d.get('k_begin', 0)
        p.k_count = d.get('k_count', A.shape[0] if d.get('rows') is None else d['rows'].shape[0])
    oa = (_lib.WgradOutput * len(outputs))()
    for d, o in zip(outputs, oa):
        o.kind, o.n_groups, o.first_problem = d.get('kind', WGRAD_PLAIN), d.get('n_groups', 1), d['first_problem']
        C = _chk(d['C'])
        o.C, o.ldc = C.data_ptr() + 4 * d.get('c_offset', 0), d.get('ldc', C.shape[-1])
        o.c_split, o.c_delta = d.get('c_split', 0), d.get('c_delta', 0)
        o.n_scalers, o.scaler_stride = d.get('n_scalers', 1), d.get('scaler_stride', 0)
        o.aff = d['aff'].data_ptr() if d.get('aff') is not None else None
        o.row = d['row'].data_ptr() if d.get('row') is not None else None
        if d.get('coef') is not None:
            arr = _float_array(d['coef'])
            keep.append(arr)
            o.coef = ctypes.addressof(arr)
    dev = problems[0]['A'].device
    check(L.i3d_wgrad_multi(pa, len(problems), oa, len(outputs), _p(_gemm_workspace(dev)), GEMM_WORKSPACE_BYTES, _stream()),
          'i3d_wgrad_multi')


def mha_fwd(qkv, graph_ptr, num_graphs, nhead, scale):
    _chk(qkv)
    _chk(graph_ptr, torch.int32)
    N, H = qkv.shape[0], qkv.shape[1] // 3
    out = torch.empty(N, H, dtype=torch.float32, device=qkv.device)
    lse = torch.empty(N, nhead, dtype=torch.float32, device=qkv.device)
    check(_lib.load().i3d_mha_fwd(_p(qkv), _p(graph_ptr), num_graphs, N, H, nhead, float(scale), _p(out), _p(lse), _stream()),
          'i3d_mha_fwd')
    return out, lse


def mha_bwd(qkv, out, grad_out, lse, graph_ptr, num_graphs, nhead, scale):
    for t in (qkv, out, grad_out, lse):
        _chk(t)
    N, H = out.shape
    delta = torch.empty(N, nhead, dtype=torch.float32, device=qkv.device)
    grad_qkv = torch.empty_like(qkv)
    check(_lib.load().i3d_mha_bwd(_p(qkv), _p(out), _p(grad_out), _p(lse), _p(graph_ptr), num_graphs, N, H, nhead, float(scale),
                                  _p(delta), _p(grad_qkv), _stream()), 'i3d_mha_bwd')
    return grad_qkv


def ln_res_fwd(x, r, gamma, beta, eps):
    for t in (x, r, gamma, beta):
        _chk(t)
    rows, feat = x.shape
    y = torch.empty_like(x)
    mean = torch.empty(rows, dtype=torch.float32, device=x.device)
    rstd = torch.empty(rows, dtype=torch.float32, device=x.device)
    check(_lib.load().i3d_ln_res_fwd(_p(x), _p(r), _p(gamma), _p(beta), rows, feat, float(eps), _p(y), _p(mean), _p(rstd),
                                     _stream()), 'i3d_ln_res_fwd')
    return y, mean, rstd


def ln_res_bwd(grad_y, x, r, gamma, mean, rstd):
    _chk(grad_y)
    rows, feat = x.shape
    L = _lib.load()
    gx = torch.empty_like(x)
    gg = torch.empty(feat, dtype=torch.float32, device=x.device)
    gb = torch.empty(feat, dtype=torch.float32, device=x.device)
    if rows == 0:
        return gx, gg.zero_(), gb.zero_()
    partial = torch.empty(L.i3d_ln_res_partial_floats(rows, feat), dtype=torch.float32, device=x.device)
    check(L.i3d_ln_res_bwd(_p(grad_y), _p(x), _p(r), _p(gamma), _p(mean), _p(rstd), rows, feat, _p(gx), _p(partial), _p(gg),
                           _p(gb), _stream()), 'i3d_ln_res_bwd')
    return gx, gg, gb


def pair_sum_fwd(u, bias, pidx):
    _chk(u)
    _chk(bias)
    P, feat = pidx.num_edges, u.shape[1]
    out = torch.empty(P, feat, dtype=torch.float32, device=u.device)
    check(_lib.load().i3d_pair_sum_fwd(_p(u), _p(bias), _p(pidx.src_s), _p(pidx.dst_s), _p(pidx.perm), P, feat, _p(out),
                                       _stream()), 'i3d_pair_sum_fwd')
    return out


def pair_sum_bwd(grad_out, u, bias, pidx):
    _chk(grad_out)
    P, feat = pidx.num_edges, u.shape[1]
    gp = torch.empty(P, feat, dtype=torch.float32, device=u.device)
    check(_lib.load().i3d_pair_sum_bwd(_p(grad_out), _p(u), _p(bias), _p(pidx.src_s), _p(pidx.dst_s), _p(pidx.perm), P, feat,
                                       _p(gp), _stream()), 'i3d_pair_sum_bwd')
    return _pair_node_sums(gp, gp, pidx)


def pair_norm_fwd(p, pidx):
    _chk(p)
    P = pidx.num_edges
    out = torch.empty(P, 1, dtype=torch.float32, device=p.device)
    check(_lib.load().i3d_pair_norm_fwd(_p(p), _p(pidx.src_s), _p(pidx.dst_s), _p(pidx.perm), P, p.shape[1], _p(out),
                                        _stream()), 'i3d_pair_norm_fwd')
    return out


def pair_norm_bwd(grad_out, p, dist, pidx):
    _chk(grad_out)
    P, feat = pidx.num_edges, p.shape[1]
    gp = torch.empty(P, 2 * feat, dtype=torch.float32, device=p.device)
# ... 752 lines not shown
```

3dinfomax_amd/pna_native.py:

```python
import ctypes
import os

import torch

from . import _lib, ops, streams, tape

NATIVE_MODEL = os.environ.get('I3D_NATIVE_MODEL', '1') != '0'
_SIMPLE = (None, 'relu', 'leakyrelu')
_MAX_GROUPS, _MAX_COEF = _lib.array_len(_lib.GroupedFcArgs, 'group_start'), _lib.array_len(_lib.GroupedFcArgs, 'coef')


class _Desc:
    __slots__ = ('struct', 'params', 'param_ids', 'keep', 'grad_key', 'fcs', 'bn_feat', 'target_dim', 'emb_params')


def _fc_ok(fc, need_bn):
    if not fc.bias:
        return False
    if fc.dropout is not None:
        return False
    if fc.batch_norm is None:
        return not need_bn and fc.activation in _SIMPLE
    return (fc.activation in _SIMPLE and fc.sync_group is None and fc.batch_norm.affine
            and fc.batch_norm.track_running_stats and fc.batch_norm.momentum is not None)


def eligible(module, g):
    if not NATIVE_MODEL:
        return False
    if not module.training and torch.is_grad_enabled():
        return False
    if tape.active() is not None:
        return False
    from . import layers as _layers
    from . import pna as P
    if not P.EDGE_TABLE:
        return False
    plist = tape._param_list(module)
    ent = module.__dict__.get('_i3d_native_ok')
    if ent is None or ent[0] is not plist:
        from .layers import FCLayer
        ent = module.__dict__['_i3d_native_ok'] = (plist, _structure_ok(module),
                                                   [m for m in module.modules() if isinstance(m, FCLayer)])
    if not ent[1]:
        return False
    for fc in ent[2]:
        if fc.sync_group is not None:
            return False
    for fc in ent[2]:
        bn = fc.batch_norm
        if fc.training != module.training or (bn is not None and bn.training != module.training):
            return False
    if module.training and not _layers._composite_ok(ent[2][0].hot()[4]):
        return False
    feat = g.ndata.get('feat')
    ef = g.edata.get('feat')
    if feat is None or ef is None or not feat.is_cuda or feat.dtype != torch.int64 or ef.dtype != torch.int64:
        return False
    idx = g.index()
    if idx.num_edges == 0 or idx.num_nodes == 0:
        return False
    groups = idx.degree_groups()[2]
    n_sc = len(module.node_gnn.mp_layers[0].scalers)
    return len(groups) <= _MAX_GROUPS and len(groups) * n_sc <= _MAX_COEF


def _structure_ok(module):
    gnn = module.node_gnn
    if len(gnn.mp_layers) < 1 or len(gnn.mp_layers) > 16:
        return False
    first = gnn.mp_layers[0]
    hidden = gnn.atom_encoder.atom_embedding_list[0].embedding_dim
    if hidden % 4 or len(first.scalers) < 2 or not first.edge_features:
        return False
    if getattr(gnn.atom_encoder, 'padding', False) or getattr(gnn.bond_encoder, 'padding', False):
        return False
    n_comb = 1
    for d in gnn.bond_encoder.dims:
        n_comb *= d
    if n_comb > 256 or len(gnn.bond_encoder.dims) > 8 or len(gnn.atom_encoder.dims) > 16:
        return False
    for layer in gnn.mp_layers:
        if layer.pairwise_distances:
            return False
        pre, post = list(layer.pretrans.fully_connected), list(layer.posttrans.fully_connected)
        if len(post) != 1 or not 1 <= len(pre) <= 4:
            return False
        if layer.aggregators != first.aggregators or layer.scalers != first.scalers or layer.residual != first.residual:
            return False
        if float(layer.avg_d['log']) != float(first.avg_d['log']):
            return False
# ... 127 lines not shown

    @staticmethod
    def forward(ctx, module, g, state, *params):
        gnn = module.node_gnn
        idx = g.index()
        dev = idx.in_ptr.device
        desc = module.__dict__.get('_i3d_desc_fwd')
        ids = tuple(id(p) for p in params)
        if desc is None or desc.param_ids != ids:
            desc = _describe(module)
            desc.param_ids = ids
            module.__dict__['_i3d_desc_fwd'] = desc
        desc.struct.training = 1 if module.training else 0
        atom_feat, bond_feat = g.ndata['feat'].contiguous(), g.edata['feat'].contiguous()
        b, comb = _batch_struct(g, idx, gnn)
        b.atom_feat, b.bond_feat = atom_feat.data_ptr(), bond_feat.data_ptr()
        L = _lib.load()
        n_saved = L.i3d_pna_model_saved_floats(ctypes.byref(desc.struct), ctypes.byref(b))
        if n_saved < 0:
            _lib.check(1, 'i3d_pna_model_saved_floats')
        N, E, B, F = idx.num_nodes, idx.num_edges, idx.num_graphs, desc.struct.hidden
        saved = torch.empty(n_saved, dtype=torch.float32, device=dev)
        node_emb = torch.empty(N, F, dtype=torch.float32, device=dev)
        edge_emb = torch.empty(E, F, dtype=torch.float32, device=dev)
        out = torch.empty(B, desc.target_dim, dtype=torch.float32, device=dev)
        events = None
        if ops.KERNEL_TIMERS is not None:
            nl = desc.struct.n_layers
            evs = [ops.RawEvent() for _ in range(2 * nl)]
            events = (ctypes.c_void_p * (2 * nl))(*[e.handle for e in evs])
            f_msg = gnn.mp_layers[0].pretrans.fully_connected[-1].out_dim
            for l in range(nl):
                ops.KERNEL_TIMERS.setdefault('pna_aggregate_fwd', []).append(
                    (evs[2 * l], evs[2 * l + 1], N, E, f_msg, desc.struct.n_aggregators * f_msg))
        handle = ctypes.c_void_p()
        _lib.check(L.i3d_pna_model_fwd(ctypes.byref(desc.struct), ctypes.byref(b), saved.data_ptr(), node_emb.data_ptr(),
                                       edge_emb.data_ptr(), out.data_ptr(), ops._workspace(desc.bn_feat, dev).data_ptr(), events,
                                       ops._stream(), ctypes.byref(handle)), 'i3d_pna_model_fwd')
        ctx.handle = _CtxHandle(handle.value)
        ctx.keep = (saved, node_emb, atom_feat, bond_feat, comb, idx, desc)
        ctx.module, ctx.state, ctx.params, ctx.batch = module, state, params, b
        ctx.mark_non_differentiable(node_emb, edge_emb)
        ctx.set_materialize_grads(False)
        return out, node_emb, edge_emb

    @staticmethod
    def backward(ctx, grad, _g_node, _g_edge):
        if grad is None:
            return (None,) * (3 + len(ctx.params))
        streams.invalidate_step()
        module, params = ctx.module, ctx.params
        dev = grad.device
        direct = tape.DIRECT_PARAM_GRADS and tape._plain_leaves(params)
        if direct and tape.PERSISTENT_GRADS:
            pool = ctx.state.pool_for(params)
            views, key = pool.view_of, ('pool', id(pool))
        else:
            sizes = [p.numel() for p in params]
            flat = torch.empty(sum(sizes), dtype=torch.float32, device=dev)
            views, key = {id(p): v.view_as(p) for p, v in zip(params, flat.split(sizes))}, None
        at, bt = ctx.keep[6].emb_params
        if not (_contiguous_views(at, views) and _contiguous_views(bt, views)):
            views = dict(views)
            for tabs in (at, bt):
                blk = torch.empty(sum(t.shape[0] for t in tabs), tabs[0].shape[1], dtype=torch.float32, device=dev)
                o = 0
                for t in tabs:
                    views[id(t)] = blk[o:o + t.shape[0]]
                    o += t.shape[0]
            key = None
        desc = module.__dict__.get('_i3d_desc_bwd') if key is not None else None
        ids = tuple(id(p) for p in params)
        if desc is None or desc.grad_key != key or desc.param_ids != ids:
            desc = _describe(module, views)
            desc.grad_key, desc.param_ids = key, ids
            if key is not None:
                module.__dict__['_i3d_desc_bwd'] = desc
        L = _lib.load()
        n_scratch = L.i3d_pna_model_scratch_floats(ctypes.byref(desc.struct), ctypes.byref(ctx.batch))
        scratch = torch.empty(n_scratch, dtype=torch.float32, device=dev)
        grad = grad.contiguous()
        bn_ws, gemm_ws = ops._workspace(desc.bn_feat, dev).data_ptr(), ops._gemm_workspace(dev).data_ptr()

        def part(k, split):
            _lib.check(L.i3d_pna_model_bwd_part(ctx.handle.ptr, ctypes.byref(desc.struct), grad.data_ptr(), scratch.data_ptr(), bn_ws,
                                                gemm_ws, ops.GEMM_WORKSPACE_BYTES, k, split, ops._stream()), 'i3d_pna_model_bwd_part')

        red = ctx.state.reducer
        n_layers = desc.struct.n_layers
        if (red is not None and red._agreed and n_layers >= 2 and key is not None
                and ctx.state.sink_views is views and (_world(red.group) > 1 or _FORCE_EARLY)):
            split = n_layers // 2
            part(1, split)
            red.launch_async(module)
            part(2, split)
        else:
            part(0, 0)
        out = [views[id(p)] for p in params]
        sink = ctx.state.sink
        if sink is not None:
            out = sink(params, out)
        ctx.keep = ctx.handle = None
        if direct:
            for p, gr in zip(params, out):
                p.grad = gr
            return (None,) * (3 + len(params))
        return (None, None, None) + tuple(out)


_FORCE_EARLY = _lib.TEST_HOOKS['force_early_allreduce']


def _world(group):
    import torch.distributed as dist
    return dist.get_world_size(group) if dist.is_initialized() else 1


def run(module, g):
    params = [p for p in tape._param_list(module) if p.requires_grad]
    if len(params) != len(tape._param_list(module)):
        return None
    out, node_emb, edge_emb = PNAModelFn.apply(module, g, tape.model_state(module), *params)
    g.ndata['feat'] = node_emb
    g.edata['feat'] = edge_emb
    return out


def debug_messages(out, layer, num_edges, feat):
    node = out.grad_fn
    handle = getattr(node, 'handle', None)
    if handle is None:
        raise RuntimeError('not the output of the native PNA sequencer (or its backward pass has already run)')
    msg = torch.empty(num_edges, feat, dtype=torch.float32, device=out.device)
    _lib.check(_lib.load().i3d_pna_model_debug_messages(handle.ptr, layer, msg.data_ptr(), ops._stream()),
               'i3d_pna_model_debug_messages')
    return msg
```

include/infomax3d_hip.h:

```cpp
#ifndef INFOMAX3D_HIP_H
#define INFOMAX3D_HIP_H

#include <stdint.h>

#ifdef __cplusplus
extern "C" {
#endif

#define I3D_OK 0
#define I3D_ERR_INVALID (-1)
#define I3D_ERR_LAUNCH (-2)
#define I3D_NOT_TAKEN 1

#define I3D_ACT_NONE 0
#define I3D_ACT_RELU 1
#define I3D_ACT_SILU 2
#define I3D_ACT_SIGMOID 3
#define I3D_ACT_LEAKY_RELU 4
#define I3D_ACT_TANH 5
#define I3D_ACT_ELU 6
#define I3D_ACT_SELU 7
#define I3D_ACT_SOFTPLUS 8

#define I3D_AGG_MEAN 0
#define I3D_AGG_SUM 1
#define I3D_AGG_MAX 2
#define I3D_AGG_MIN 3
#define I3D_AGG_STD 4
#define I3D_AGG_VAR 5

#define I3D_SCALE_IDENTITY 0
#define I3D_SCALE_AMPLIFICATION 1
#define I3D_SCALE_ATTENUATION 2

int i3d_abi_version(void);
const char* i3d_last_error(void);

int i3d_embedding_sum_fwd(const int64_t* idx, const int* row_perm, int rows, int n_cols, const float* const* tables,
                          int feat, float* out, void* stream);
int i3d_embedding_sum_bwd(const int64_t* idx, const int* row_perm, int rows, int n_cols, const float* grad_out,
                          int feat, float* const* grad_tables, const int* dims, void* stream);

int i3d_pna_aggregate_fwd(const float* e, const int* in_ptr, int num_nodes, int feat, const int* aggregators,
                          int n_aggregators, const int* scalers, int n_scalers, int force_scalers, float avg_d_log,
                          float* out, void* stream);
int i3d_pna_aggregate_bwd(const float* grad_out, const float* e, const int* in_ptr, int num_nodes, int feat,
                          const int* aggregators, int n_aggregators, const int* scalers, int n_scalers,
                          int force_scalers, float avg_d_log, float* grad_e, void* stream);

int i3d_segment_readout_fwd(const float* x, const int* graph_ptr, int num_graphs, int feat, const int* ops,
                            int n_ops, float* out, void* stream);
int i3d_segment_readout_bwd(const float* grad_out, const float* x, const int* graph_ptr, int num_graphs, int feat,
                            const int* ops, int n_ops, float* grad_x, void* stream);

int i3d_gemm_f32(int trans_a, int trans_b, int M, int N, int K, const float* A, int lda, const float* B, int ldb,
                 float* C, int ldc, const float* bias, int accumulate, void* stream);
int i3d_gemm_f32_ex(int trans_a, int trans_b, int M, int N, int K, const float* A, int lda, const float* B, int ldb,
                    float* C, int ldc, const float* bias, int accumulate, int tile_cfg, int splits, void* workspace,
                    long workspace_bytes, void* stream);
int i3d_set_matmul_precision(int bf16);
int i3d_get_matmul_precision(void);
int i3d_set_fp32_products(int split);
int i3d_get_fp32_products(void);

long i3d_panel_packed_bytes(int N, int K);
int i3d_panel_pack(const float* W, int ldw, int N, int K, int trans, void* packed, void* stream);
typedef struct {
    const float* W;
    int ldw, N, K, trans;
    void* packed;
} I3dPanelPack;
int i3d_panel_pack_multi(const I3dPanelPack* weights, int n, void* stream);
int i3d_panel_gemm(int M, int N, int K, const float* A, int lda, const void* packed, float* C, int ldc, const float* bias,
                   int accumulate, void* stream);
int i3d_panel_stats_tiles(int M);
int i3d_panel_gemm_fused(int M, int N, int K, const float* A, int lda, const void* packed, float* C, int ldc, const float* bias,
                         const float* a_aff, int epi_act, float* stats, void* stream);

int i3d_gemm_f32_ws(int trans_a, int trans_b, int M, int N, int K, const float* A, int lda, const float* B, int ldb,
                    float* C, int ldc, const float* bias, int accumulate, void* workspace, long workspace_bytes,
                    void* stream);

int i3d_gemm_f32_blocks(int trans_a, int trans_b, int M, int N, int K, const float* A, int lda, const float* B, int ldb,
                        int b_split, long b_delta, long b_view_floats, float* C, int ldc, int c_split, long c_delta,
                        int accumulate, void* workspace, long workspace_bytes, void* stream);

int i3d_pna_aggregate_fwd_towers(const float* e, const int* in_ptr, int num_nodes, int feat, int tower_feat,
                                 const int* aggregators, int n_aggregators, const int* scalers, int n_scalers,
                                 int force_scalers, float avg_d_log, float* out, void* stream);
int i3d_pna_aggregate_bwd_towers(const float* grad_out, const float* e, const int* in_ptr, int num_nodes, int feat,
                                 int tower_feat, const int* aggregators, int n_aggregators, const int* scalers,
                                 int n_scalers, int force_scalers, float avg_d_log, float* grad_e, void* stream);
int i3d_gemm_f32_batched(int trans_a, int trans_b, int M, int N, int K, const float* A, int lda, long a_batch, const float* B,
                         int ldb, long b_batch, float* C, int ldc, long c_batch, int n_batch, int accumulate, void* workspace,
                         long workspace_bytes, void* stream);

int i3d_gemm_f32_grouped_batched(int trans_b, int m_padded, int N, int K, const float* A, int lda, long a_batch, long a_rows_total,
                                 const int* m_rows, const int* tile_group, const float* B, int ldb, long b_group_stride, long b_batch,
                                 float* C, int ldc, long c_batch, int n_batch, int accumulate, void* stream);

int i3d_pna_combine_weights_fwd(const float* W, int ldw, int f_in, int f_out, int agg_width, int n_groups,
                                int n_scalers, const float* coef, float* WD, void* stream);
int i3d_pna_combine_weights_bwd(const float* dWD, int ldw, int f_in, int f_out, int agg_width, int n_groups,
                                int n_scalers, const float* coef, float* dW, void* stream);
int i3d_gemm_f32_grouped(int trans_b, int m_padded, int N, int K, const float* A, int lda, long a_rows_total,
                         const int* m_rows, const int* tile_group, const float* B, int ldb, long b_group_stride,
                         float* C, int ldc, int accumulate, void* stream);
int i3d_gemm_f32_rowsubset(int M, int N, int n_rows, const float* A, int lda, const float* B, int ldb,
                           const int* k_rows, long rows_total, float* C, int ldc, int accumulate, void* stream);
int i3d_gemm_f32_rowsubset_multi(int M, int N, int n_groups, const int* group_start, const int* group_count,
                                 const float* A, int lda, const float* B, int ldb, const int* k_rows, long rows_total,
                                 float* C, long c_group_stride, int ldc, int accumulate, int tile_cfg, int seg_rows,
                                 void* workspace, long workspace_bytes, void* stream);

long i3d_colreduce_workspace_bytes(int rows, int feat);
int i3d_act_stats_fwd(const float* pre, int rows, int feat, int act, float* x, float eps, float momentum,
                      float* mean, float* invstd, float* running_mean, float* running_var, double* sums_out,
// ... 129 lines not shown
int i3d_tower_layer_bwd(const I3dTowerLayerArgs* a, void* stream);

int i3d_bn_finalize_partials(const float* partial, int n_tiles, int feat, float eps, float momentum, const float* gamma,
                             const float* beta, float* mean, float* invstd, float* running_mean, float* running_var,
                             long long* num_batches_tracked, float* aff, void* stream);
int i3d_edge_stats_rows_per_tile(int feat);
int i3d_edge_combine_act_stats(const float* P, int ldp, const float* Q, const int* q_code, const float* bias,
                               const int* src_s, const int* dst_s, int num_edges, int feat, int act, float* x,
                               float* partial, void* stream);
int i3d_gemm_f32_fused(int M, int N, int K, const float* A, int lda, long a_rows_total, const float* W, int ldb, float* C,
                       int ldc, const float* bias, int accumulate, const float* a_aff, int epi_act, float* stats,
                       const int* m_rows, const int* tile_group, long b_group_stride, void* stream);
int i3d_gemm_f32_fused_src(int M, int N, int K, const float* A, int lda, long a_rows_total, const float* W, int ldb, float* C,
                           int ldc, const float* c_in, int ldcin, const float* bias, int accumulate, const float* a_aff,
                           int epi_act, float* stats, const int* m_rows, const int* tile_group, long b_group_stride,
                           void* stream);
int i3d_gemm_f32_fused_bf16out(int M, int N, int K, const float* A, int lda, long a_rows_total, const float* W, int ldb, void* C, int ldc,
                               const float* bias, const float* a_aff, int epi_act, float* stats, void* stream);
int i3d_pna_pack_h_weights(const float* W_edge, int ldw_edge, int f_out_edge, const float* W_post, int ldw_post, int f_out_post,
                           const float* bias_post, int f_h, float* Wcat, float* bcat, void* stream);
int i3d_bn_bwd_strided(const float* grad_y, const float* x, const float* pre, int rows, int feat, int act, int post_act,
                       const float* mean, const float* invstd, const float* gamma, const float* beta, float* grad_gamma,
                       float* grad_beta, float* grad_pre, int ld_out, float* grad_bias, void* workspace, void* stream);
int i3d_bn_bwd_x_bf16(const float* grad_y, const void* x, int rows, int feat, int act, int post_act, const float* mean,
                      const float* invstd, const float* gamma, const float* beta, float* grad_gamma, float* grad_beta, float* grad_pre,
                      float* grad_bias, void* workspace, void* stream);
int i3d_gemm_f32_wgrad_bn(int f_out, int f_in, int rows, const float* dY, int ldy, const float* x, int ldx, float* dW,
                          int ldw, const float* grad_bias, const float* aff, void* workspace, long workspace_bytes,
                          void* stream);
typedef struct {
    int world;
    int (*all_gather_f32)(void* user, const float* send, float* recv, long count, void* stream);
    int (*all_reduce_f64)(void* user, double* buf, long count, void* stream);
    void* user;
    void* scratch;
    long scratch_bytes;
} I3dCollectives;
int i3d_set_collectives(const I3dCollectives* c );
int i3d_collectives_world(void);
int i3d_collectives_all_gather_f32(const float* send, float* recv, long count, void* stream);
int i3d_collectives_all_reduce_f64(double* buf, long count, void* stream);
int i3d_rccl_available(void);
int i3d_rccl_unique_id(char* out128 );
int i3d_rccl_init(const char* id128 , int rank, int world, void** comm);
int i3d_rccl_destroy(void* comm);
int i3d_set_collectives_rccl(void* comm, int world, void* scratch, long scratch_bytes);
long i3d_peer_mailbox_bytes(void);
int i3d_peer_handle_bytes(void);
int i3d_peer_alloc(void** mailbox , char* handle_out );
int i3d_peer_free(void* mailbox);
int i3d_peer_open(void* mailbox, const char* handles , int rank, int world,
                  double timeout_s , void** ctx );
int i3d_set_collectives_peer(void* ctx, void* scratch, long scratch_bytes);
int i3d_peer_bind_stream(void* ctx, void* stream, void* scratch, long scratch_bytes);
int i3d_peer_status(void* ctx);
long long i3d_peer_sequence(void* ctx);
int i3d_peer_close(void* ctx);

#define I3D_WGRAD_PLAIN 0
#define I3D_WGRAD_BN 1
#define I3D_WGRAD_COMBINE 2
typedef struct {
    const float* A;
    const float* B;
    const int* rows;
    long rows_total;
    int lda, ldb, M, N;
    int k_begin, k_count;
} I3dWgradProblem;
typedef struct {
    int kind, n_groups, first_problem;
    int ldc, c_split, n_scalers;
    long c_delta, scaler_stride;
    float* C;
    const float* aff;
    const float* row;
    const float* coef;
} I3dWgradOutput;
int i3d_wgrad_multi_supported(const I3dWgradProblem* problems, int n_problems, const I3dWgradOutput* outputs, int n_outputs);
long i3d_wgrad_multi_workspace_bytes(int max_units);
long i3d_wgrad_multi_min_workspace_bytes(const I3dWgradProblem* problems, int n_problems);
int i3d_wgrad_multi(const I3dWgradProblem* problems, int n_problems, const I3dWgradOutput* outputs, int n_outputs,
                    void* workspace, long workspace_bytes, void* stream);

int i3d_pna_aggregate_fwd_aff(const float* e, const float* aff, const int* in_ptr, int num_nodes, int feat,
                              const int* aggregators, int n_aggregators, const int* scalers, int n_scalers,
                              int force_scalers, float avg_d_log, float* out, void* stream);
int i3d_pna_aggregate_bwd_aff(const float* grad_out, const float* e, const float* aff, const int* in_ptr, int num_nodes,
                              int feat, const int* aggregators, int n_aggregators, const int* scalers, int n_scalers,
                              int force_scalers, float avg_d_log, float* grad_e, void* stream);
int i3d_pna_aggregate_fwd_ex(const void* e, int e_bf16, const float* aff, const int* in_ptr, int num_nodes, int feat,
                             const int* aggregators, int n_aggregators, const int* scalers, int n_scalers, int force_scalers,
                             float avg_d_log, float* out, void* stream);
int i3d_pna_aggregate_bwd_ex(const float* grad_out, const void* e, int e_bf16, const float* aff, const int* in_ptr, int num_nodes,
                             int feat, const int* aggregators, int n_aggregators, const int* scalers, int n_scalers,
                             int force_scalers, float avg_d_log, float* grad_e, void* stream);

int i3d_set_bn_bwd_one_launch(int on);
int i3d_bn_bwd_one_launch_supported(int rows, int feat);
long i3d_bn_bias_partial_floats(int feat);
int i3d_bn_bwd_edge_sums(const float* grad_y, const float* x, int rows, int feat, int act, const float* mean, const float* invstd,
                         const float* gamma, const float* beta, float* grad_gamma, float* grad_beta, float* grad_pre,
                         const int* in_ptr, const int* out_ptr, const int* out_epos, int num_nodes, float* out_src, float* out_dst,
                         int ldo, void* workspace, void* stream);
int i3d_colsum_strided(const float* x, int ldx, int rows, int feat, float* out, float* partial, void* stream);

typedef struct {
    int act, post_act;
    float eps, momentum;
    const float* gamma;
    const float* beta;
    float* running_mean;
    float* running_var;
    float* mean;
    float* invstd;
    void* workspace;
    void* gemm_workspace;
    long gemm_workspace_bytes;
    long long* num_batches_tracked;
} I3dBnTail;

typedef struct {
    I3dBnTail tail;
    int rows, f_in, f_out, ldw;
    const float* x;
    const float* W;
    const float* bias;
    const float* residual;
    float* xact;
    float* pre_keep;
    float* y;
    const float* grad_y;
    float* grad_pre;
    float* grad_gamma;
    float* grad_beta;
    float* grad_W;
    float* grad_bias;
    float* grad_x;
    void* W_dgrad_panel;
    void* W_fwd_panel;
} I3dFcArgs;

typedef struct {
    I3dBnTail tail;
    int num_nodes, num_edges, f_h, f_q, f_out, ldw;
    int q_rows;
    int v_pad;
    const int* q_code;
    const float* onehot;
    float* grad_Q;
    const float* h;
    const float* q;
    const float* W;
    const float* bias;
    const int* src_s;
    const int* dst_s;
    const int* in_ptr;
    const int* out_ptr;
    const int* out_epos;
    float* P;
    float* Q;
    float* xact;
    float* pre_keep;
    float* y;
    const float* grad_y;
    float* grad_pre;
    float* grad_P;
    float* grad_gamma;
    float* grad_beta;
    float* grad_W;
    float* grad_bias;
    float* grad_h;
    float* grad_q;
    int grad_q_accumulate;
} I3dEdgeFcArgs;

typedef struct {
    I3dBnTail tail;
    int num_nodes, f_h, f_out, agg_width, ldw, n_groups, n_scalers, m_padded;
    int group_start[32];
    int group_count[32];
    float coef[128];
// ... 46 lines not shown
    float* Wcat;
    float* bcat;
    float* PL;
    float* DL;
    int wgrad_split;
    int eval_mode;
    int msg_bf16;
    float* edge_bias_partial;
    void* Wcat_panel;
    void* Wcat_dgrad_panel;
} I3dPnaLayerArgs;

typedef struct {
    const float* running_mean;
    const float* running_var;
    const float* gamma;
    const float* beta;
    float* aff;
    int feat;
    float eps;
} I3dBnEvalAff;
int i3d_bn_eval_aff_multi(const I3dBnEvalAff* entries , int n, void* stream);

long i3d_pna_layer_stats_floats(int num_nodes, int num_edges, int m_padded, int f);

typedef struct {
    I3dBnTail tail_in;
    I3dBnTail tail_msg;
    int num_nodes, num_edges, hidden, n_enc, reduce_mean;
    int ld_w_in, ld_w_msg;
    const float* d_raw;
    const int* perm;
    const int* dst_s;
    const int* in_ptr;
    const float* emb;
    const float* W_in;
    const float* b_in;
    const float* W_msg;
    const float* b_msg;
    const float* w_gate;
    const float* b_gate;
    float* stats;
    float* aff_in;
    float* aff_msg;
    float* x_msg;
    float* d_out;
    float* msg;
    float* m_sum;
    const float* grad_m_sum;
    float* grad_ya;
    float* grad_lin;
    float* partial;
    float* grad_W_in;
    float* grad_b_in;
    float* grad_gamma_in;
    float* grad_beta_in;
    float* grad_W_msg;
    float* grad_b_msg;
    float* grad_gamma_msg;
    float* grad_beta_msg;
    float* grad_w_gate;
    float* grad_b_gate;
    float* grad_emb;
    int store_bf16;
    float* x_center;
} I3dNet3dEdgeArgs;
int i3d_net3d_edge_supported(int hidden, int n_enc);
long i3d_net3d_edge_stats_floats(int num_edges, int hidden);
long i3d_net3d_edge_bwd_floats(int num_edges, int hidden, int n_enc);
int i3d_net3d_edge_fwd(const I3dNet3dEdgeArgs* args, void* stream);
int i3d_net3d_edge_bwd(const I3dNet3dEdgeArgs* args, void* stream);

int i3d_event_create(void** event);
int i3d_event_destroy(void* event);
int i3d_event_record(void* event, void* stream);
int i3d_event_elapsed_ms(void* start, void* stop, float* ms);

int i3d_wgrad_stream_join(void* stream);
int i3d_wgrad_stream_fork(void* stream, void** side);
int i3d_wgrad_stream_peek(void* stream, void** side);
int i3d_pna_layer_weights_fwd(const I3dPnaLayerArgs* args, void* stream);
int i3d_pna_layer_fwd(const I3dPnaLayerArgs* args, void* stream);
int i3d_pna_layer_bwd(const I3dPnaLayerArgs* args, void* stream);
int i3d_fc_bn_fwd(const I3dFcArgs* args, void* stream);
int i3d_fc_bn_bwd(const I3dFcArgs* args, void* stream);
int i3d_fc_bn_bwd_chain(const I3dFcArgs* args, void* stream);
int i3d_fc_bn_bwd_wgrad(const I3dFcArgs* args, void* stream);
int i3d_edge_fc_bn_fwd(const I3dEdgeFcArgs* args, void* stream);
int i3d_edge_fc_bn_bwd(const I3dEdgeFcArgs* args, void* stream);
int i3d_grouped_fc_bn_fwd(const I3dGroupedFcArgs* args, void* stream);
int i3d_grouped_fc_bn_bwd(const I3dGroupedFcArgs* args, void* stream);

#define I3D_MAX_LAYERS 16
#define I3D_MAX_HEAD_FC 4
typedef struct {
    const float* W;
    const float* bias;
    const float* gamma;
    const float* beta;
    float* running_mean;
    float* running_var;
    long long* num_batches_tracked;
    float* grad_W;
    float* grad_bias;
    float* grad_gamma;
    float* grad_beta;
    int f_in, f_out, act;
    float eps, momentum;
} I3dFcParams;

typedef struct {
    int training;
    int n_layers, hidden, n_pre, residual;
    int n_aggregators, aggregators[8];
    int n_scalers, scalers[4];
    float avg_d_log;
    I3dFcParams pre[I3D_MAX_LAYERS][I3D_MAX_EXTRA_FC + 1];
    I3dFcParams post[I3D_MAX_LAYERS];
    int n_atom_tables, atom_dims[16];
    const float* atom_tables[16];
    float* grad_atom_tables;
    int n_bond_tables, bond_dims[16];
    const float* bond_tables[16];
    float* grad_bond_tables;
    int n_readout, readout_ops[4];
    int n_head;
    I3dFcParams head[I3D_MAX_HEAD_FC];
} I3dPnaModel;

typedef struct {
    int num_nodes, num_edges, num_graphs;
    const int64_t* atom_feat;
    const int64_t* bond_feat;
    const int* in_ptr;
    const int* perm;
    const int* src_s;
    const int* dst_s;
    const int* out_ptr;
    const int* out_epos;
    const int* graph_ptr;
    const int* deg_rows;
    const int* deg_tile_group;
    int m_padded, n_groups;
    int group_degree[32], group_start[32], group_count[32];
    const int64_t* comb;
    int n_comb, v_pad;
} I3dPnaBatch;

long i3d_pna_model_saved_floats(const I3dPnaModel* model, const I3dPnaBatch* batch);
long i3d_pna_model_scratch_floats(const I3dPnaModel* model, const I3dPnaBatch* batch);
int i3d_pna_model_fwd(const I3dPnaModel* model, const I3dPnaBatch* batch, float* saved, float* node_emb, float* edge_emb,
                      float* out, void* bn_workspace, void* const* agg_events, void* stream, void** ctx_out);
int i3d_pna_model_bwd(void* ctx, const I3dPnaModel* grads_from, const float* grad_out, float* scratch, void* bn_workspace,
                      void* gemm_workspace, long gemm_workspace_bytes, void* stream);
int i3d_pna_model_bwd_part(void* ctx, const I3dPnaModel* grads_from, const float* grad_out, float* scratch, void* bn_workspace,
                           void* gemm_workspace, long gemm_workspace_bytes, int part, int split, void* stream);
int i3d_pna_model_ctx_free(void* ctx);
int i3d_pna_messages_normalized(const float* e, const float* aff, long rows, int feat, float* out, void* stream);
int i3d_pna_messages_normalized_ex(const void* e, int e_bf16, const float* aff, long rows, int feat, float* out, void* stream);
int i3d_pna_model_debug_messages(void* ctx, int layer, float* out, void* stream);

int i3d_adam_chunk_elems(void);
int i3d_adam_chunk_bytes(void);
int i3d_adam_step(const void* chunk_table, int n_chunks, float* steps, int n_steps, double lr, double beta1, double beta2,
                  double weight_decay, double eps, double bias_correction1, double bias_correction2_sqrt, void* stream);

// ... 237 lines not shown
```

Measured before the change: 274,400.

## Deduplicate PNA weight-gradient chunks for degree-one groups and gate fused BN bwd on residency

```diff
diff --git a/3dinfomax_amd/csrc/bn.hip b/3dinfomax_amd/csrc/bn.hip
--- a/3dinfomax_amd/csrc/bn.hip
+++ b/3dinfomax_amd/csrc/bn.hip
@@ -1,5 +1,6 @@
 #include <stdlib.h>
 
+#include <algorithm>
 #include <atomic>
 
 #include "common.h"
@@ -1022,17 +1023,54 @@
            (long)rows <= (long)FUSED_MAX_BLOCKS * (FUSED_THREADS / (feat / 4)) * FUSED_MAX_RPT;
 }
 
+static int fused_resident_blocks() {
+    constexpr int MAX_DEV = 64, SIMD_VGPRS = 512;
+    static std::atomic<int> cache[MAX_DEV];
+    int dev = -1;
+    if (hipGetDevice(&dev) != hipSuccess || dev < 0 || dev >= MAX_DEV) { (void)hipGetLastError(); return 0; }
+    const int known = cache[dev].load(std::memory_order_relaxed);
+    if (known != 0) return known > 0 ? known : 0;
+    int cus = 0, lds_cu = 0, per_cu = 0, total = -1;
+    hipFuncAttributes at;
+    int panel_regs = 0, panel_lds = 0;
+    if (hipDeviceGetAttribute(&cus, hipDeviceAttributeMultiprocessorCount, dev) == hipSuccess &&
+        hipDeviceGetAttribute(&lds_cu, hipDeviceAttributeMaxSharedMemoryPerMultiprocessor, dev) == hipSuccess &&
+        hipOccupancyMaxActiveBlocksPerMultiprocessor(&per_cu, reinterpret_cast<const void*>(&bn_bwd_fused_kernel<8, true>), FUSED_THREADS, 0) == hipSuccess &&
+        hipFuncGetAttributes(&at, reinterpret_cast<const void*>(&bn_bwd_fused_kernel<8, true>)) == hipSuccess &&
+        wgrad_panel_footprint(&panel_regs, &panel_lds)) {
+        const int waves_per_simd = FUSED_THREADS / 64 / 4;
+        const int regs = std::max((at.numRegs + 7) / 8 * 8, 8), lds = std::max((int)at.sharedSizeBytes, 1);
+        const int by_regs = (SIMD_VGPRS - (panel_regs + 7) / 8 * 8) / (waves_per_simd * regs);
+        const int by_lds = (lds_cu - panel_lds) / lds;
+        per_cu = std::max(0, std::min(per_cu, std::min(by_regs, by_lds)));
+        total = (long)cus * per_cu > 0 ? (int)std::min<long>((long)cus * per_cu, 1 << 30) : -1;
+    } else {
+        (void)hipGetLastError();
+    }
+    cache[dev].store(total, std::memory_order_relaxed);
+    return total > 0 ? total : 0;
+}
+
+static int one_launch_grid(int rows, int feat, int* rows_per_block) {
+    const int rl = FUSED_THREADS / (feat / 4);
+    int G = cdiv(rows, rl);
+    if (G > FUSED_MAX_BLOCKS) G = FUSED_MAX_BLOCKS;
+    const int rpb = cdiv(rows, G);
+    if (rows_per_block != nullptr) *rows_per_block = rpb;
+    return cdiv(rows, rpb);
+}
+
+static bool one_launch_resident(int rows, int feat) { return one_launch_grid(rows, feat, nullptr) <= fused_resident_blocks(); }
+
 static bool bn_bwd_one_launch(const BwdApplyArgs& b, int rows, int feat, void* workspace, float* grad_beta, float* grad_gamma, hipStream_t s) {
     if (!g_one_launch || !fused_final() || !one_launch_shape(rows, feat) || b.pre != nullptr || b.grad_pre == nullptr) return false;
+    if (!one_launch_resident(rows, feat)) return false;
     if (b.ld_out % 4 != 0 || ((((uintptr_t)b.grad_y) | ((uintptr_t)b.grad_pre)) & 15) != 0 || (((uintptr_t)b.x) & (b.x_bf16 ? 7 : 15)) != 0)
         return false;
     FusedBwdGeom ge;
     ge.tpr = feat / 4;
     ge.rl = FUSED_THREADS / ge.tpr;
-    int G = cdiv(rows, ge.rl);
-    if (G > FUSED_MAX_BLOCKS) G = FUSED_MAX_BLOCKS;
-    ge.rpb = cdiv(rows, G);
-    G = cdiv(rows, ge.rpb);
+    const int G = one_launch_grid(rows, feat, &ge.rpb);
     unsigned tag = ++g_fused_tag;
     if (tag == 0) tag = ++g_fused_tag;
     ge.tag = tag;
@@ -1208,8 +1246,10 @@
 }
 
 extern "C" int i3d_bn_bwd_one_launch_supported(int rows, int feat) {
-    return g_one_launch && fused_final() && collectives() == nullptr && one_launch_shape(rows, feat) ? 1 : 0;
-}
+    return g_one_launch && fused_final() && collectives() == nullptr && one_launch_shape(rows, feat) && one_launch_resident(rows, feat) ? 1 : 0;
+}
+
+extern "C" int i3d_bn_bwd_one_launch_resident_blocks(void) { return fused_resident_blocks(); }
 
 extern "C" int i3d_set_bn_bwd_one_launch(int on) {
     const int was = g_one_launch;
diff --git a/3dinfomax_amd/csrc/common.h b/3dinfomax_amd/csrc/common.h
--- a/3dinfomax_amd/csrc/common.h
+++ b/3dinfomax_amd/csrc/common.h
@@ -29,6 +29,7 @@
     } while (0)
 
 static inline int cdiv(long a, long b) { return (int)((a + b - 1) / b); }
+bool wgrad_panel_footprint(int* vgprs, int* lds_bytes);
 
 constexpr int WAVE = 64;
 
diff --git a/3dinfomax_amd/csrc/composite.hip b/3dinfomax_amd/csrc/composite.hip
--- a/3dinfomax_amd/csrc/composite.hip
+++ b/3dinfomax_amd/csrc/composite.hip
@@ -281,7 +281,7 @@
            a->edge_bias_partial != nullptr && e->grad_bias != nullptr;
 }
 
-static int pna_layer_wgrad_multi(const I3dPnaLayerArgs* a, void* wst, bool dry_run, int part = 0) {
+static int pna_layer_wgrad_multi(const I3dPnaLayerArgs* a, const int* group_degree, void* wst, bool dry_run, int part = 0) {
     static const bool on = [] { const char* e = getenv("I3D_WGRAD_MULTI"); return e == nullptr || e[0] != '0'; }();
     const I3dEdgeFcArgs* e = &a->edge;
     const I3dGroupedFcArgs* g = &a->post;
@@ -296,12 +296,19 @@
     constexpr int MAX_PROBLEMS = 40, MAX_OUTPUTS = 8, MAX_GROUPS = 32, MAX_SCALERS = 4;
     I3dWgradProblem pr[MAX_PROBLEMS];
     I3dWgradOutput out[MAX_OUTPUTS];
+    int dup[MAX_PROBLEMS * I3D_WGRAD_DUP_INTS];
     float coef[MAX_GROUPS * MAX_SCALERS];
+    const int f_msg = a->n_pre_extra > 0 ? a->pre[a->n_pre_extra - 1].f_out : e->f_out;
+    const bool dedup = group_degree != nullptr && i3d_get_wgrad_dedup() != 0 && a->n_aggregators == 4 &&
+                       a->aggregators[0] == I3D_AGG_MEAN && a->aggregators[1] == I3D_AGG_MAX && a->aggregators[2] == I3D_AGG_MIN &&
+                       a->aggregators[3] == I3D_AGG_STD && A == 4 * f_msg && f_msg % 4 == 0 && f_msg >= 4 && f_msg <= 208;
+    bool any_dup = false;
     const int fixed_problems = 3 + (a->n_pre_extra > 0 ? a->n_pre_extra : 0);
     if (g->n_scalers > MAX_SCALERS || g->n_scalers < 0 || fixed_problems >= MAX_PROBLEMS || 4 + a->n_pre_extra > MAX_OUTPUTS) return 0;
     const int max_group_problems = MAX_PROBLEMS - fixed_problems < MAX_GROUPS ? MAX_PROBLEMS - fixed_problems : MAX_GROUPS;
     std::memset(pr, 0, sizeof(pr));
     std::memset(out, 0, sizeof(out));
+    std::memset(dup, 0, sizeof(dup));
     int np = 0, no = 0;
     auto problem = [&](const float* Ap, int lda, int M, const float* Bp, int ldb, int Nn, long rows_total, const int* rows,
                        int k_begin, int k_count) {
@@ -327,6 +334,14 @@
             if (ng >= max_group_problems) return 0;
             for (int s = 0; s < g->n_scalers; ++s) coef[ng * g->n_scalers + s] = g->coef[k * g->n_scalers + s];
             problem(dlin, ld_dlin, g->f_out, g->agg, A, A, N, g->deg_rows, g->group_start[k], g->group_count[k]);
+            if (dedup) {
+                int* const d = dup + (np - 1) * I3D_WGRAD_DUP_INTS;
+                const bool one = group_degree[k] == 1;
+                d[I3D_WGRAD_DUP_WIDTH] = f_msg;
+                for (int c = 0; c < I3D_WGRAD_DUP_CHUNKS; ++c) d[I3D_WGRAD_DUP_SRC + c] = (one && c < 3) ? 0 : c;
+                d[I3D_WGRAD_DUP_UNIFORM] = one ? 1 << 3 : 0;
+                any_dup = any_dup || one;
+            }
             ++ng;
         }
         if (ng == 0) return 0;
@@ -354,11 +369,13 @@
     }
     void* ws = e->tail.gemm_workspace;
     const long wsb = e->tail.gemm_workspace_bytes;
-    if (ws == nullptr || !i3d_wgrad_multi_supported(pr, np, out, no) || i3d_wgrad_multi_min_workspace_bytes(pr, np) > wsb) return 0;
+    const int* dups = any_dup ? dup : nullptr;
+    if (ws == nullptr || !i3d_wgrad_multi_dup_supported(pr, np, dups, out, no) || i3d_wgrad_multi_dup_min_workspace_bytes(pr, dups, np) > wsb)
+        return 0;
     if (dry_run) return 1;
     if (do_pre && edge_bwd_fused_ok(a) && !edge_bias_on_chain(a))
         TRY(i3d_colsum_strided(a->DL + Fo, 2 * Fo + a->post.f_out, N, Fo, e->grad_bias, a->edge_bias_partial, wst));
-    TRY(i3d_wgrad_multi(pr, np, out, no, ws, wsb, wst));
+    TRY(i3d_wgrad_multi_dup(pr, np, dups, out, no, ws, wsb, wst));
     if (!do_pre) return 1;
     const int V = e->q_rows;
     TRY(i3d_gemm_f32_ws(1, 0, Fo, e->f_q, V, e->grad_Q, Fo, e->q, e->f_q, e->grad_W + 2 * Fh, e->ldw, nullptr, 0, ws, wsb, wst));
@@ -367,7 +384,7 @@
     return 1;
 }
 
-static bool wgrad_multi_layer_ok(const I3dPnaLayerArgs* a);
+static bool wgrad_multi_layer_ok(const I3dPnaLayerArgs* a, const int* group_degree);
 
 static bool simple_act(int act) { return act == I3D_ACT_NONE || act == I3D_ACT_RELU || act == I3D_ACT_LEAKY_RELU; }
 
@@ -497,14 +514,14 @@
     return I3D_OK;
 }
 
-extern "C" int i3d_pna_layer_bwd(const I3dPnaLayerArgs* a, void* stream) {
+static int pna_layer_bwd(const I3dPnaLayerArgs* a, const int* group_degree, void* stream) {
     I3D_CHECK_ARG(a != nullptr && a->n_pre_extra >= 0 && a->n_pre_extra <= I3D_MAX_EXTRA_FC && a->n_post_extra >= 0 &&
                       a->n_post_extra <= I3D_MAX_EXTRA_FC, "bad arguments");
     Aux* x = aux_for((hipStream_t)stream);
     for (int i = a->n_post_extra - 1; i >= 0; --i) TRY(fc_bn_bwd_chain(&a->postx[i], stream));
     const bool inplace = a->residual && a->post.grad_h == a->grad_out && a->n_post_extra == 0;
     I3D_CHECK_ARG(a->post.grad_h != a->grad_out || inplace, "grad_h may alias grad_out only for a residual layer without extra blocks");
-    const bool multi = wgrad_multi_layer_ok(a);
+    const bool multi = wgrad_multi_layer_ok(a, group_degree);
     const bool merged = multi && merge_h_ok(a) && a->DL != nullptr;
     const long n = (long)a->edge.num_nodes * a->edge.f_h;
     if (merged) {
@@ -523,7 +540,7 @@
     void* wst = stream;
     if (multi && a->wgrad_split) {
         wst = fork_wgrad(x, stream);
-        const int took = pna_layer_wgrad_multi(a, wst, false, 1);
+        const int took = pna_layer_wgrad_multi(a, group_degree, wst, false, 1);
         if (took < 0) return took;
         I3D_CHECK_ARG(took == 1, "weight-gradient launch refused a layer it had accepted");
     }
@@ -566,7 +583,7 @@
             TRY(edge_fc_bn_bwd_sums(&a->edge, stream));
         }
         wst = fork_wgrad(x, stream);
-        const int took = pna_layer_wgrad_multi(a, wst, false, a->wgrad_split ? 2 : 0);
+        const int took = pna_layer_wgrad_multi(a, group_degree, wst, false, a->wgrad_split ? 2 : 0);
         if (took < 0) return took;
         I3D_CHECK_ARG(took == 1, "weight-gradient launch refused a layer it had accepted");
     } else {
@@ -595,7 +612,15 @@
     return join_wgrad(x, stream);
 }
 
-static bool wgrad_multi_layer_ok(const I3dPnaLayerArgs* a) { return pna_layer_wgrad_multi(a, nullptr, true) == 1; }
+static bool wgrad_multi_layer_ok(const I3dPnaLayerArgs* a, const int* group_degree) {
+    return pna_layer_wgrad_multi(a, group_degree, nullptr, true) == 1;
+}
+
+extern "C" int i3d_pna_layer_bwd(const I3dPnaLayerArgs* a, void* stream) { return pna_layer_bwd(a, nullptr, stream); }
+
+extern "C" int i3d_pna_layer_bwd_deg(const I3dPnaLayerArgs* a, const int* group_degree, void* stream) {
+    return pna_layer_bwd(a, group_degree, stream);
+}
 
 extern "C" int i3d_wgrad_stream_join(void* stream) { return join_wgrad(aux_for((hipStream_t)stream), stream); }
 
diff --git a/3dinfomax_amd/csrc/embedding.hip b/3dinfomax_amd/csrc/embedding.hip
--- a/3dinfomax_amd/csrc/embedding.hip
+++ b/3dinfomax_amd/csrc/embedding.hip
@@ -124,7 +124,7 @@
 
 using namespace i3d;
 
-extern "C" int i3d_abi_version(void) { return 2; }
+extern "C" int i3d_abi_version(void) { return I3D_ABI_VERSION; }
 
 extern "C" const char* i3d_last_error(void) { return g_err; }
 
diff --git a/3dinfomax_amd/csrc/model.hip b/3dinfomax_amd/csrc/model.hip
--- a/3dinfomax_amd/csrc/model.hip
+++ b/3dinfomax_amd/csrc/model.hip
@@ -524,7 +524,7 @@
         a.edge_bias_partial = sd.take(i3d_bn_bias_partial_floats(e.f_out));
         e.grad_q = grad_table;
         e.grad_q_accumulate = (l == L - 1) ? 0 : 1;
-        TRY(i3d_pna_layer_bwd(&a, stream));
+        TRY(i3d_pna_layer_bwd_deg(&a, c->b.group_degree, stream));
         c->gh_cur = nxt;
         if (leaves_pending) {
             void* wst = stream;
diff --git a/3dinfomax_amd/csrc/wgrad.hip b/3dinfomax_amd/csrc/wgrad.hip
--- a/3dinfomax_amd/csrc/wgrad.hip
+++ b/3dinfomax_amd/csrc/wgrad.hip
@@ -1,6 +1,7 @@
 #include "common.h"
 
 #include <algorithm>
+#include <atomic>
 #include <cstdlib>
 #include <cstring>
 
@@ -46,7 +47,14 @@
     int m_chunks, n_chunks;
     int k_begin, k_end, k_per_slice;
     int unit_begin;
+    int n_comp, mapped;
+    unsigned comp_map, uniform;
 };
+
+__device__ __forceinline__ int wg_nvalid(const WgProb& p, const int nc) {
+    const int nv = min(p.ncw, p.N - nc * p.ncw);
+    return (p.mapped && ((p.uniform >> nc) & 1u)) ? min(nv, 16) : nv;
+}
 
 struct WgArgs {
     float* slab;
@@ -76,7 +84,7 @@
     const int l15 = lane & 15, lk = lane >> 4;
     const int k0 = p.k_begin + slice * p.k_per_slice;
     const int klen = min(p.k_end - k0, p.k_per_slice);
-    const int mvalid = min(p.mcw, p.M - mc * p.mcw), nvalid = min(p.ncw, p.N - nc * p.ncw);
+    const int mvalid = min(p.mcw, p.M - mc * p.mcw), nvalid = wg_nvalid(p, nc);
     const int mtl = (mvalid + 15) / 16, ntl = NFULL ? WG_T : (nvalid + 15) / 16;
 
     for (int i = threadIdx.x; i < klen; i += 256) kidx[i] = p.rows != nullptr ? p.rows[k0 + i] : k0 + i;
@@ -265,9 +273,10 @@
     while (pi + 1 < a.n_problems && a.p[pi + 1].unit_begin <= u) ++pi;
     const WgProb& p = a.p[pi];
     const int local = u - p.unit_begin;
-    const int nc = local % p.n_chunks, mc = (local / p.n_chunks) % p.m_chunks, slice = local / (p.n_chunks * p.m_chunks);
+    const int j = local % p.n_comp, mc = (local / p.n_comp) % p.m_chunks, slice = local / (p.n_comp * p.m_chunks);
+    const int nc = p.mapped ? (int)((p.comp_map >> (4 * j)) & 15u) : j;
     float* out = a.slab + (long)u * WG_UNIT_FLOATS;
-    const int mvalid = min(p.mcw, p.M - mc * p.mcw), nvalid = min(p.ncw, p.N - nc * p.ncw);
+    const int mvalid = min(p.mcw, p.M - mc * p.mcw), nvalid = wg_nvalid(p, nc);
     const int mtl = (mvalid + 15) / 16;
     const bool nfull = nvalid > 192;
 #ifdef WG_TIMING
@@ -310,6 +319,8 @@
     WgOut o[WG_MAX_OUTPUTS];
     int unit_begin[WG_MAX_PROBLEMS];
     int n_slices[WG_MAX_PROBLEMS];
+    int n_comp[WG_MAX_PROBLEMS];
+    unsigned slot_map[WG_MAX_PROBLEMS], uniform[WG_MAX_PROBLEMS];
     float coef[32][4];
 };
 
@@ -331,8 +342,14 @@
     for (int g = 0; g < o.n_groups; ++g) {
         const int pi = o.first_problem + g;
         const int zn = a.n_slices[pi];
-        const long stride = (long)o.m_chunks * o.n_chunks * WG_UNIT_FLOATS;
-        const float* p = a.slab + ((long)a.unit_begin[pi] + (long)mc * o.n_chunks + nc) * WG_UNIT_FLOATS + tile * 256 + lane * 4;
+        int per = o.n_chunks, slot = nc, tl = tile;
+        if (a.n_comp[pi] > 0) {
+            per = a.n_comp[pi];
+            slot = (int)((a.slot_map[pi] >> (4 * nc)) & 15u);
+            if ((a.uniform[pi] >> nc) & 1u) tl = mt * WG_T;
+        }
+        const long stride = (long)o.m_chunks * per * WG_UNIT_FLOATS;
+        const float* p = a.slab + ((long)a.unit_begin[pi] + (long)mc * per + slot) * WG_UNIT_FLOATS + tl * 256 + lane * 4;
         float4 v = make_float4(0.f, 0.f, 0.f, 0.f);
         constexpr int FL = 8;
         for (int z0 = 0; z0 < zn; z0 += FL) {
@@ -401,16 +418,80 @@
     return cdiv(cdiv(n, chunks), 4) * 4;
 }
 
+struct NGeo {
+    int ncw, n_chunks, n_comp;
+    bool mapped;
+    unsigned comp_map, slot_map, uniform_k, uniform_r;
+};
+
+bool n_geometry(const I3dWgradProblem& p, const int* d, NGeo& g) {
+    g.ncw = chunk_width(p.N, g.n_chunks);
+    g.n_comp = g.n_chunks;
+    g.mapped = false;
+    g.comp_map = g.slot_map = g.uniform_k = g.uniform_r = 0;
+    if (d == nullptr || d[I3D_WGRAD_DUP_WIDTH] == 0) return true;
+    const int w = d[I3D_WGRAD_DUP_WIDTH], umask = d[I3D_WGRAD_DUP_UNIFORM];
+    const int* const src = d + I3D_WGRAD_DUP_SRC;
+    if (w < 4 || w > WG_LD || w % 4 != 0 || p.N < 4) return false;
+    const int nch = cdiv(p.N, w);
+    if (nch > I3D_WGRAD_DUP_CHUNKS || umask < 0 || (umask >> nch) != 0) return false;
+    int slot_of[I3D_WGRAD_DUP_CHUNKS];
+    g.ncw = w; g.n_chunks = nch; g.n_comp = 0; g.mapped = true;
+    for (int c = 0; c < nch; ++c) {
+        const int s = src[c];
+        if (s < 0 || s >= nch || src[s] != s) return false;
+        if (s != c && (std::min(w, p.N - c * w) != std::min(w, p.N - s * w) || ((umask >> c) & 1))) return false;
+        if (s == c) {
+            slot_of[c] = g.n_comp;
+            g.comp_map |= (unsigned)c << (4 * g.n_comp);
+            ++g.n_comp;
+        }
+    }
+    for (int c = 0; c < nch; ++c) {
+        const int s = src[c];
+        g.slot_map |= (unsigned)slot_of[s] << (4 * c);
+        if ((umask >> s) & 1) g.uniform_r |= 1u << c;
+    }
+    g.uniform_k = (unsigned)umask;
+    return true;
+}
+
+std::atomic<int> g_dedup_on{1};
+std::atomic<long> g_dedup_launches{0};
+
+}
+
+bool wgrad_panel_footprint(int* vgprs, int* lds_bytes) {
+    hipFuncAttributes at;
+    if (hipFuncGetAttributes(&at, reinterpret_cast<const void*>(&wgrad_multi_kernel<PREC_F32>)) != hipSuccess) return false;
+    *vgprs = at.numRegs;
+    *lds_bytes = (int)at.sharedSizeBytes;
+    return true;
 }
 }
 
 using namespace i3d;
 
-extern "C" int i3d_wgrad_multi_supported(const I3dWgradProblem* problems, int n_problems, const I3dWgradOutput* outputs,
-                                         int n_outputs) {
+extern "C" int i3d_set_wgrad_dedup(int on) { return g_dedup_on.exchange(on != 0); }
+extern "C" int i3d_get_wgrad_dedup(void) { return g_dedup_on.load(); }
+extern "C" long i3d_wgrad_dedup_launches(void) { return g_dedup_launches.load(); }
+
+extern "C" int i3d_wgrad_multi_dup_supported(const I3dWgradProblem* problems, int n_problems, const int* dups,
+                                             const I3dWgradOutput* outputs, int n_outputs) {
     if (problems == nullptr || outputs == nullptr || n_problems < 1 || n_problems > WG_MAX_PROBLEMS || n_outputs < 1 ||
         n_outputs > WG_MAX_OUTPUTS)
         return 0;
+    for (int i = 0; i < n_problems; ++i) {
+        const I3dWgradProblem& p = problems[i];
+        if (p.A == nullptr || p.B == nullptr || p.M < 4 || p.N < 4 || p.M % 4 != 0 || p.N % 4 != 0 || p.lda % 4 != 0 ||
+            p.ldb % 4 != 0 || p.lda < p.M || p.ldb < p.N || ((((uintptr_t)p.A) | ((uintptr_t)p.B)) & 15) != 0 || p.k_count < 0 ||
+            p.rows_total < 1)
+            return 0;
+        if (((p.rows_total - 1) * p.lda + p.M) * 4 >= (1L << 32) - 16 || ((p.rows_total - 1) * p.ldb + p.N) * 4 >= (1L << 32) - 16)
+            return 0;
+        NGeo g;
+        if (!n_geometry(p, dups != nullptr ? dups + i * I3D_WGRAD_DUP_INTS : nullptr, g)) return 0;
+    }
     int combines = 0;
     for (int i = 0; i < n_outputs; ++i) {
         const I3dWgradOutput& o = outputs[i];
@@ -424,18 +505,20 @@
         if (o.C == nullptr || o.ldc % 4 != 0 || o.c_delta % 4 != 0 || (((uintptr_t)o.C) & 15) != 0) return 0;
         if (o.kind == I3D_WGRAD_BN && (o.aff == nullptr || o.row == nullptr || (((uintptr_t)o.aff) & 15) != 0)) return 0;
         if (o.first_problem < 0 || o.first_problem + o.n_groups > n_problems) return 0;
+        NGeo g0, g;
+        n_geometry(problems[o.first_problem], dups != nullptr ? dups + o.first_problem * I3D_WGRAD_DUP_INTS : nullptr, g0);
+        for (int k = 1; k < o.n_groups; ++k) {
+            n_geometry(problems[o.first_problem + k], dups != nullptr ? dups + (o.first_problem + k) * I3D_WGRAD_DUP_INTS : nullptr, g);
+            if (g.ncw != g0.ncw || g.n_chunks != g0.n_chunks) return 0;
+        }
     }
     if (combines > 1) return 0;
-    for (int i = 0; i < n_problems; ++i) {
-        const I3dWgradProblem& p = problems[i];
-        if (p.A == nullptr || p.B == nullptr || p.M < 4 || p.N < 4 || p.M % 4 != 0 || p.N % 4 != 0 || p.lda % 4 != 0 ||
-            p.ldb % 4 != 0 || p.lda < p.M || p.ldb < p.N || ((((uintptr_t)p.A) | ((uintptr_t)p.B)) & 15) != 0 || p.k_count < 0 ||
-            p.rows_total < 1)
-            return 0;
-        if (((p.rows_total - 1) * p.lda + p.M) * 4 >= (1L << 32) - 16 || ((p.rows_total - 1) * p.ldb + p.N) * 4 >= (1L << 32) - 16)
-            return 0;
-    }
     return 1;
+}
+
+extern "C" int i3d_wgrad_multi_supported(const I3dWgradProblem* problems, int n_problems, const I3dWgradOutput* outputs,
+                                         int n_outputs) {
+    return i3d_wgrad_multi_dup_supported(problems, n_problems, nullptr, outputs, n_outputs);
 }
 
 static int problem_kps(const I3dWgradProblem& p, int kps) {
@@ -447,78 +530,121 @@
     return (int)std::min<long>(WG_MAX_SLICE, scaled / WG_BK * WG_BK);
 }
 
-static long plan_units(const I3dWgradProblem* problems, int n, int kps) {
+static long plan_units(const I3dWgradProblem* problems, const int* dups, int n, int kps) {
     long u = 0;
     for (int i = 0; i < n; ++i) {
-        int mch, nch;
+        int mch;
+        NGeo g;
         chunk_width(problems[i].M, mch);
-        chunk_width(problems[i].N, nch);
-        u += (long)mch * nch * cdiv(problems[i].k_count, problem_kps(problems[i], kps));
+        if (!n_geometry(problems[i], dups != nullptr ? dups + i * I3D_WGRAD_DUP_INTS : nullptr, g)) return 1L << 40;
+        u += (long)mch * g.n_comp * cdiv(problems[i].k_count, problem_kps(problems[i], kps));
     }
     return u;
 }
 
 extern "C" long i3d_wgrad_multi_workspace_bytes(int max_units) { return (long)max_units * WG_UNIT_FLOATS * 4; }
 
+extern "C" long i3d_wgrad_multi_dup_min_workspace_bytes(const I3dWgradProblem* problems, const int* dups, int n_problems) {
+    if (problems == nullptr || n_problems < 1) return -1;
+    return (plan_units(problems, dups, n_problems, WG_MAX_SLICE) + 1) * (long)WG_UNIT_FLOATS * 4 + (1 << 16);
+}
+
 extern "C" long i3d_wgrad_multi_min_workspace_bytes(const I3dWgradProblem* problems, int n_problems) {
-    if (problems == nullptr || n_problems < 1) return -1;
-    return (plan_units(problems, n_problems, WG_MAX_SLICE) + 1) * (long)WG_UNIT_FLOATS * 4 + (1 << 16);
-}
-
-extern "C" int i3d_wgrad_multi(const I3dWgradProblem* problems, int n_problems, const I3dWgradOutput* outputs, int n_outputs,
-                               void* workspace, long workspace_bytes, void* stream) {
-    I3D_CHECK_ARG(i3d_wgrad_multi_supported(problems, n_problems, outputs, n_outputs), "unsupported problem set");
+    return i3d_wgrad_multi_dup_min_workspace_bytes(problems, nullptr, n_problems);
+}
+
+static long make_plan(const I3dWgradProblem* problems, const int* dups, int n_problems, long max_units, WgArgs& a,
+                      WgReduceArgs& r, bool& dedup) {
+    static const int fixed_rows = env_int("I3D_WGRAD_ROWS", 0) / WG_BK * WG_BK;
+    static const int target_units = env_int("I3D_WGRAD_UNITS", 256);
+    int kps;
+    if (fixed_rows > 0) {
+        kps = std::min(WG_MAX_SLICE, fixed_rows);
+        while (kps < WG_MAX_SLICE && plan_units(problems, nullptr, n_problems, kps) > max_units) kps = std::min(WG_MAX_SLICE, kps * 2);
+    } else {
+        const long target = std::min<long>(max_units, target_units);
+        int lo = 128 / WG_BK, hi = WG_MAX_SLICE / WG_BK;
+        while (lo < hi) {
+            const int mid = (lo + hi) / 2;
+            if (plan_units(problems, nullptr, n_problems, mid * WG_BK) <= target) hi = mid;
+            else lo = mid + 1;
+        }
+        kps = lo * WG_BK;
+    }
+    while (dups != nullptr && kps < WG_MAX_SLICE && plan_units(problems, dups, n_problems, kps) > max_units) kps += WG_BK;
+    if (plan_units(problems, dups, n_problems, kps) > max_units) return -1;
+    a.n_problems = n_problems;
+    dedup = false;
+    long units = 0;
+    for (int i = 0; i < n_problems; ++i) {
+        const I3dWgradProblem& s = problems[i];
+        WgProb& p = a.p[i];
+        NGeo g;
+        if (!n_geometry(s, dups != nullptr ? dups + i * I3D_WGRAD_DUP_INTS : nullptr, g)) return -1;
+        p.A = s.A; p.B = s.B; p.rows = s.rows;
+        p.a_bytes = (unsigned)(((s.rows_total - 1) * s.lda + s.M) * 4);
+        p.b_bytes = (unsigned)(((s.rows_total - 1) * s.ldb + s.N) * 4);
+        p.lda = s.lda; p.ldb = s.ldb; p.M = s.M; p.N = s.N;
+        p.mcw = chunk_width(s.M, p.m_chunks);
+        p.ncw = g.ncw; p.n_chunks = g.n_chunks;
+        p.n_comp = g.n_comp; p.mapped = g.mapped ? 1 : 0; p.comp_map = g.comp_map; p.uniform = g.uniform_k;
+        p.k_begin = s.k_begin; p.k_end = s.k_begin + s.k_count;
+        const int n_slices = cdiv(s.k_count, problem_kps(s, kps));
+        p.k_per_slice = n_slices > 0 ? cdiv(cdiv(s.k_count, n_slices), WG_BK) * WG_BK : WG_BK;
+        p.unit_begin = (int)units;
+        r.unit_begin[i] = (int)units;
+        r.n_slices[i] = s.k_count > 0 ? cdiv(s.k_count, p.k_per_slice) : 0;
+        r.n_comp[i] = g.mapped ? g.n_comp : 0;
+        r.slot_map[i] = g.slot_map;
+        r.uniform[i] = g.uniform_r;
+        dedup = dedup || g.n_comp < g.n_chunks || g.uniform_k != 0;
+        units += (long)p.m_chunks * g.n_comp * r.n_slices[i];
+    }
+    if (units > max_units) return -1;
+    a.n_units = (int)units;
+    return units;
+}
+
+extern "C" int i3d_wgrad_multi_plan(const I3dWgradProblem* problems, const int* dups, int n_problems, long workspace_bytes,
+                                    int* unit_begin, int* n_slices, int* k_per_slice, int* n_comp, int* slot, int* first_tile) {
+    I3D_CHECK_ARG(problems != nullptr && n_problems >= 1 && n_problems <= WG_MAX_PROBLEMS && unit_begin != nullptr && n_slices != nullptr &&
+                      k_per_slice != nullptr && n_comp != nullptr && slot != nullptr && first_tile != nullptr, "bad arguments");
+    WgArgs a;
+    WgReduceArgs r;
+    bool dedup;
+    const long units = make_plan(problems, dups, n_problems, workspace_bytes / ((long)WG_UNIT_FLOATS * 4), a, r, dedup);
+    I3D_CHECK_ARG(units >= 0, "description not valid or scratch too small");
+    for (int i = 0; i < n_problems; ++i) {
+        unit_begin[i] = r.unit_begin[i]; n_slices[i] = r.n_slices[i]; k_per_slice[i] = a.p[i].k_per_slice; n_comp[i] = a.p[i].n_comp;
+        for (int c = 0; c < I3D_WGRAD_DUP_CHUNKS; ++c) {
+            const bool in = c < a.p[i].n_chunks;
+            slot[i * I3D_WGRAD_DUP_CHUNKS + c] = !in ? -1 : (a.p[i].mapped ? (int)((r.slot_map[i] >> (4 * c)) & 15u) : c);
+            first_tile[i * I3D_WGRAD_DUP_CHUNKS + c] = in ? (int)((r.uniform[i] >> c) & 1u) : 0;
+        }
+    }
+    return (int)units;
+}
+
+extern "C" int i3d_wgrad_multi_dup(const I3dWgradProblem* problems, int n_problems, const int* dups, const I3dWgradOutput* outputs,
+                                   int n_outputs, void* workspace, long workspace_bytes, void* stream) {
+    I3D_CHECK_ARG(i3d_wgrad_multi_dup_supported(problems, n_problems, dups, outputs, n_outputs), "unsupported problem set");
     I3D_CHECK_ARG(workspace != nullptr && (((uintptr_t)workspace) & 15) == 0, "scratch required");
 #ifdef WG_TIMING
     const long max_units = (workspace_bytes - (1 << 16)) / ((long)WG_UNIT_FLOATS * 4);
 #else
     const long max_units = workspace_bytes / ((long)WG_UNIT_FLOATS * 4);
 #endif
-    static const int fixed_rows = env_int("I3D_WGRAD_ROWS", 0) / WG_BK * WG_BK;
-    static const int target_units = env_int("I3D_WGRAD_UNITS", 256);
-    int kps;
-    if (fixed_rows > 0) {
-        kps = std::min(WG_MAX_SLICE, fixed_rows);
-        while (kps < WG_MAX_SLICE && plan_units(problems, n_problems, kps) > max_units) kps = std::min(WG_MAX_SLICE, kps * 2);
-    } else {
-        const long target = std::min<long>(max_units, target_units);
-        int lo = 128 / WG_BK, hi = WG_MAX_SLICE / WG_BK;
-        while (lo < hi) {
-            const int mid = (lo + hi) / 2;
-            if (plan_units(problems, n_problems, mid * WG_BK) <= target) hi = mid;
-            else lo = mid + 1;
-        }
-        kps = lo * WG_BK;
-    }
-    I3D_CHECK_ARG(plan_units(problems, n_problems, kps) <= max_units, "scratch too small");
     WgArgs a;
     WgReduceArgs r;
+    bool dedup = false;
+    const long planned = make_plan(problems, dups, n_problems, max_units, a, r, dedup);
+    I3D_CHECK_ARG(planned >= 0, "scratch too small");
+    const int units = (int)planned;
     a.slab = (float*)workspace;
     a.stamps = nullptr;
 #ifdef WG_TIMING
     a.stamps = (unsigned long long*)((char*)workspace + workspace_bytes - (1 << 16));
 #endif
-    a.n_problems = n_problems;
-    int units = 0;
-    for (int i = 0; i < n_problems; ++i) {
-        const I3dWgradProblem& s = problems[i];
-        WgProb& p = a.p[i];
-        p.A = s.A; p.B = s.B; p.rows = s.rows;
-        p.a_bytes = (unsigned)(((s.rows_total - 1) * s.lda + s.M) * 4);
-        p.b_bytes = (unsigned)(((s.rows_total - 1) * s.ldb + s.N) * 4);
-        p.lda = s.lda; p.ldb = s.ldb; p.M = s.M; p.N = s.N;
-        p.mcw = chunk_width(s.M, p.m_chunks);
-        p.ncw = chunk_width(s.N, p.n_chunks);
-        p.k_begin = s.k_begin; p.k_end = s.k_begin + s.k_count;
-        const int n_slices = cdiv(s.k_count, problem_kps(s, kps));
-        p.k_per_slice = n_slices > 0 ? cdiv(cdiv(s.k_count, n_slices), WG_BK) * WG_BK : WG_BK;
-        p.unit_begin = units;
-        r.unit_begin[i] = units;
-        r.n_slices[i] = s.k_count > 0 ? cdiv(s.k_count, p.k_per_slice) : 0;
-        units += p.m_chunks * p.n_chunks * r.n_slices[i];
-    }
-    I3D_CHECK_ARG(units <= max_units, "scratch too small");
-    a.n_units = units;
     hipStream_t st = (hipStream_t)stream;
     if (units > 0) {
         const char* const sb = getenv("I3D_WGRAD_SPLIT_BF16");
@@ -528,6 +654,7 @@
         else if (prec == PREC_BF16X3) hipLaunchKernelGGL(wgrad_multi_kernel<PREC_BF16X3>, dim3(units), dim3(256), 0, st, a);
         else hipLaunchKernelGGL(wgrad_multi_kernel<PREC_F32>, dim3(units), dim3(256), 0, st, a);
         I3D_CHECK_LAUNCH();
+        if (dedup) g_dedup_launches.fetch_add(1);
     }
     r.slab = a.slab;
     r.n_outputs = n_outputs;
@@ -555,3 +682,8 @@
     I3D_CHECK_LAUNCH();
     return I3D_OK;
 }
+
+extern "C" int i3d_wgrad_multi(const I3dWgradProblem* problems, int n_problems, const I3dWgradOutput* outputs, int n_outputs,
+                               void* workspace, long workspace_bytes, void* stream) {
+    return i3d_wgrad_multi_dup(problems, n_problems, nullptr, outputs, n_outputs, workspace, workspace_bytes, stream);
+}
diff --git a/3dinfomax_amd/ops.py b/3dinfomax_amd/ops.py
--- a/3dinfomax_amd/ops.py
+++ b/3dinfomax_amd/ops.py
@@ -705,6 +705,7 @@
         p.M, p.N = d.get('M', A.shape[1]), d.get('N', B.shape[1])
         p.k_begin = d.get('k_begin', 0)
         p.k_count = d.get('k_count', A.shape[0] if d.get('rows') is None else d['rows'].shape[0])
+    da = wgrad_dups(problems)
     oa = (_lib.WgradOutput * len(outputs))()
     for d, o in zip(outputs, oa):
         o.kind, o.n_groups, o.first_problem = d.get('kind', WGRAD_PLAIN), d.get('n_groups', 1), d['first_problem']
@@ -719,8 +720,23 @@
             keep.append(arr)
             o.coef = ctypes.addressof(arr)
     dev = problems[0]['A'].device
-    check(L.i3d_wgrad_multi(pa, len(problems), oa, len(outputs), _p(_gemm_workspace(dev)), GEMM_WORKSPACE_BYTES, _stream()),
-          'i3d_wgrad_multi')
+    check(L.i3d_wgrad_multi_dup(pa, len(problems), da, oa, len(outputs), _p(_gemm_workspace(dev)), GEMM_WORKSPACE_BYTES, _stream()),
+          'i3d_wgrad_multi_dup')
+
+
+def wgrad_dups(problems):
+    if not any(d.get('n_chunk_width') for d in problems):
+        return None
+    D = _lib.DEFINES
+    flat = []
+    for d in problems:
+        u = [0] * D['I3D_WGRAD_DUP_INTS']
+        u[D['I3D_WGRAD_DUP_WIDTH']], u[D['I3D_WGRAD_DUP_UNIFORM']] = d.get('n_chunk_width', 0), d.get('uniform_mask', 0)
+        src = d.get('chunk_src') or []
+        for c in range(D['I3D_WGRAD_DUP_CHUNKS']):
+            u[D['I3D_WGRAD_DUP_SRC'] + c] = src[c] if c < len(src) else c
+        flat += u
+    return _lib.int_array(flat)
 
 
 def mha_fwd(qkv, graph_ptr, num_graphs, nhead, scale):
diff --git a/3dinfomax_amd/pna_native.py b/3dinfomax_amd/pna_native.py
--- a/3dinfomax_amd/pna_native.py
+++ b/3dinfomax_amd/pna_native.py
@@ -7,6 +7,7 @@
 
 NATIVE_MODEL = os.environ.get('I3D_NATIVE_MODEL', '1') != '0'
 _SIMPLE = (None, 'relu', 'leakyrelu')
+WGRAD_DEDUP = True
 _MAX_GROUPS, _MAX_COEF = _lib.array_len(_lib.GroupedFcArgs, 'group_start'), _lib.array_len(_lib.GroupedFcArgs, 'coef')
 
 
@@ -300,6 +301,9 @@
         grad = grad.contiguous()
         bn_ws, gemm_ws = ops._workspace(desc.bn_feat, dev).data_ptr(), ops._gemm_workspace(dev).data_ptr()
 
+        if bool(L.i3d_get_wgrad_dedup()) != bool(WGRAD_DEDUP):
+            L.i3d_set_wgrad_dedup(int(bool(WGRAD_DEDUP)))
+
         def part(k, split):
             _lib.check(L.i3d_pna_model_bwd_part(ctx.handle.ptr, ctypes.byref(desc.struct), grad.data_ptr(), scratch.data_ptr(), bn_ws,
                                                 gemm_ws, ops.GEMM_WORKSPACE_BYTES, k, split, ops._stream()), 'i3d_pna_model_bwd_part')
diff --git a/include/infomax3d_hip.h b/include/infomax3d_hip.h
--- a/include/infomax3d_hip.h
+++ b/include/infomax3d_hip.h
@@ -33,6 +33,7 @@
 #define I3D_SCALE_AMPLIFICATION 1
 #define I3D_SCALE_ATTENUATION 2
 
+#define I3D_ABI_VERSION 2
 int i3d_abi_version(void);
 const char* i3d_last_error(void);
 
@@ -328,6 +329,21 @@
 long i3d_wgrad_multi_min_workspace_bytes(const I3dWgradProblem* problems, int n_problems);
 int i3d_wgrad_multi(const I3dWgradProblem* problems, int n_problems, const I3dWgradOutput* outputs, int n_outputs,
                     void* workspace, long workspace_bytes, void* stream);
+#define I3D_WGRAD_DUP_CHUNKS 8
+#define I3D_WGRAD_DUP_INTS 10
+#define I3D_WGRAD_DUP_WIDTH 0
+#define I3D_WGRAD_DUP_UNIFORM 1
+#define I3D_WGRAD_DUP_SRC 2
+int i3d_wgrad_multi_dup_supported(const I3dWgradProblem* problems, int n_problems, const int* dups,
+                                  const I3dWgradOutput* outputs, int n_outputs);
+long i3d_wgrad_multi_dup_min_workspace_bytes(const I3dWgradProblem* problems, const int* dups, int n_problems);
+int i3d_wgrad_multi_plan(const I3dWgradProblem* problems, const int* dups, int n_problems, long workspace_bytes,
+                         int* unit_begin, int* n_slices, int* k_per_slice, int* n_comp, int* slot, int* first_tile);
+int i3d_wgrad_multi_dup(const I3dWgradProblem* problems, int n_problems, const int* dups, const I3dWgradOutput* outputs,
+                        int n_outputs, void* workspace, long workspace_bytes, void* stream);
+int i3d_set_wgrad_dedup(int on);
+int i3d_get_wgrad_dedup(void);
+long i3d_wgrad_dedup_launches(void);
 
 int i3d_pna_aggregate_fwd_aff(const float* e, const float* aff, const int* in_ptr, int num_nodes, int feat,
                               const int* aggregators, int n_aggregators, const int* scalers, int n_scalers,
@@ -344,6 +360,7 @@
 
 int i3d_set_bn_bwd_one_launch(int on);
 int i3d_bn_bwd_one_launch_supported(int rows, int feat);
+int i3d_bn_bwd_one_launch_resident_blocks(void);
 long i3d_bn_bias_partial_floats(int feat);
 int i3d_bn_bwd_edge_sums(const float* grad_y, const float* x, int rows, int feat, int act, const float* mean, const float* invstd,
                          const float* gamma, const float* beta, float* grad_gamma, float* grad_beta, float* grad_pre,
@@ -556,6 +573,7 @@
 int i3d_pna_layer_weights_fwd(const I3dPnaLayerArgs* args, void* stream);
 int i3d_pna_layer_fwd(const I3dPnaLayerArgs* args, void* stream);
 int i3d_pna_layer_bwd(const I3dPnaLayerArgs* args, void* stream);
+int i3d_pna_layer_bwd_deg(const I3dPnaLayerArgs* args, const int* group_degree, void* stream);
 int i3d_fc_bn_fwd(const I3dFcArgs* args, void* stream);
 int i3d_fc_bn_bwd(const I3dFcArgs* args, void* stream);
 int i3d_fc_bn_bwd_chain(const I3dFcArgs* args, void* stream);
```

New measurement: 276,800, median of 6. Within noise of the previous version (+0.9%).
